# 10XGenomics/vartrix

Hardware: NVIDIA H100
Metric: reads_sw_scored_per_sec (higher is better)
Workload: dtype int16x2

## Files before the change

vartrix_b200/csrc/vtx_api.cu:

```cuda
#include "../../include/vartrix_b200.h"
#include "vtx_pipeline.cuh"
#include "vtx_sw.cuh"
#include "vtx_sw_band.cuh"
#include "vtx_inflate.cuh"
#include "vtx_stage.cuh"
#include "vtx_locus_stats.cuh"
#include "vtx_donors.cuh"

#include <nvtx3/nvToolsExt.h>

#include <algorithm>
#include <array>
#include <cstdarg>
#include <cstddef>
#include <cstdio>
#include <cstring>
#include <string>
#include <thread>
#include <vector>

using namespace vtx;

namespace {

thread_local std::string g_create_error;

struct Nvtx {
    explicit Nvtx(const char* name) { nvtxRangePushA(name); }
    ~Nvtx() { nvtxRangePop(); }
};
constexpr int kBandK = 6, kBandW = 20;

struct DBuf {
    void* p = nullptr;
    size_t cap = 0;
    DBuf() = default;
    DBuf(const DBuf&) = delete;
    DBuf& operator=(const DBuf&) = delete;
    ~DBuf() { release(); }
    cudaError_t release()
    {
        const cudaError_t e = p ? cudaFree(p) : cudaSuccess;
        p = nullptr; cap = 0;
        return e;
    }
    void swap(DBuf& o) { std::swap(p, o.p); std::swap(cap, o.cap); }
};

struct HostBuf {
    void* p = nullptr;
    HostBuf() = default;
    HostBuf(const HostBuf&) = delete;
    HostBuf& operator=(const HostBuf&) = delete;
    ~HostBuf() { release(); }
    void release() { if (p) cudaFreeHost(p); p = nullptr; }
    cudaError_t alloc(size_t bytes, unsigned flags = cudaHostAllocDefault)
    {
        release();
        const cudaError_t e = cudaHostAlloc(&p, bytes, flags);
        if (e != cudaSuccess) p = nullptr;
        return e;
    }
    template <typename T> T* as() const { return static_cast<T*>(p); }
};

constexpr int kResArrays = 7;
constexpr size_t kResEsz[kResArrays] = { 4, 4, 4, 4, 4, 8, 8 };

struct HostResults {
    HostBuf a[kResArrays];
    size_t cap = 0;
};

enum { EV_START = 0, EV_H2D, EV_C0, EV_PREP, EV_SW, EV_POST, EV_COUNT };

constexpr size_t kMaxCum = 4096;

struct TimeRec {
    cudaEvent_t ev[EV_COUNT] = {};
    bool had_h2d = false;
    uint64_t sw_launches = 0, launches = 0;
};

struct InSlot {
    DBuf locus_row, hap, ref_off, ref_len, alt_off, alt_len, cand_start, read_nib, read_off, read_len, cb_bytes,
        read_cb_off, read_cb_len, read_umi, cand_read;
    DBuf read_off4, read_len16, read_cb_key, cb_off_ex;
    cudaEvent_t copy_done = nullptr, free_ev = nullptr;
    bool used = false;
};

struct StageSlot {
    DBuf comp, desc, status, stream, entry, seg_count, seg_first, rec_off, rec_tid, rec_pos, rec_end, rec_fm, l_start, l_end,
        locus_row, hap, ref_off, ref_len, alt_off, alt_len, cand_count, cand_first, cand_rec, used, read_off, read_len,
        read_cb_off, read_cb_len, read_umi, cand_start, scalars, name_tab, lfilt;
    cudaEvent_t staged = nullptr, free_ev = nullptr;
    bool used_once = false;
};

}

struct vtx_ctx {
    vtx_config cfg{};
    int device = 0;
    int n_sm = 0;
    cudaStream_t stream = nullptr;
    bool own_stream = false;
    std::string err;

    DBuf bc_slot, bc_bytes, bc_off;
    DBuf bck_key, bck_idx;
    uint32_t bck_cap = 0;
    DBuf x_read_off, x_read_len, x_units, x_off4;
    DBuf band_scratch;
    DBuf inf_comp, inf_out, inf_desc, inf_status;
    bool inflate_attr_set = false;
    StageSlot sslot[2];
    uint64_t n_bam_submits = 0;
    cudaStream_t stage_stream = nullptr;
    DBuf bam_metrics;
    uint32_t min_base_quality = 0;
    DBuf stage_sums;
    bool locus_stats = false, submitted = false;
    DBuf lstats;
    size_t lstats_cap = 0;
    uint64_t stats_n = 0, stats_last_n = 0;
    HostBuf h_lstats;
    size_t h_lstats_cap = 0;
    bool donors = false;
    uint32_t n_donors = 0, donor_cols = 0, donor_last_cols = 0;
    uint64_t donor_rows = 0;
    donors::Tables donor_tab{};
    DBuf donor_dosage, donor_usable, donor_acc, donor_count, donor_start, donor_list;
    HostBuf h_donor;
    size_t h_donor_cap = 0;
    bool donor_valid = false;
    HostBuf h_stage;
    uint32_t bc_cap = 0, n_barcodes = 0;
    bool have_barcodes = false;

    InSlot slot[2];
    uint64_t n_submits = 0;
    cudaStream_t copy_stream = nullptr;
    DBuf read_col, keep, pidx, scan_sums, pair_read, pair_col, pair_umi, pair_locus, pair_start, tcount, tstart,
        pair_first, pair_cslot, pair_uslot, cslot_col, cslot_locus, uslot_cslot, ccnt, ucnt, keep2, oidx, tile_counters,
        scratch, pair_scores, d_metrics, d_res_n, big_list, slot_scratch;
    DBuf res[kResArrays];
    size_t res_cap = 0;
    size_t res_ub = 0;
    bool finished = true;
    HostResults h_res;
    HostBuf h_scalars;
    uint64_t last_n = 0;
    vtx_metrics last_metrics{};

    cudaStream_t fetch_stream = nullptr;
    HostBuf h_cum;
    unsigned long long* d_cum = nullptr;
    std::vector<TimeRec> trecs;
    size_t trec_used = 0;
    bool timing_valid = false;
    uint32_t last_tiles_nl = 0;
    bool last_tiles_valid = false;
    uint64_t t_pairs = 0;

    void* comm = nullptr;
    int rank = 0, n_ranks = 1;
    HostResults g_host;
    DBuf g_dev[kResArrays];
    DBuf g_counts;
    cudaStream_t comm_stream = nullptr;
    cudaEvent_t ev_counts = nullptr, ev_gather = nullptr, ev_results = nullptr;
    HostBuf h_counts;
    bool gather_pending = false;
    bool gather_guard = false;
    vtx_result g_out{};
};

namespace {

int set_err(vtx_ctx* c, int code, const char* fmt, ...)
{
    char buf[512];
    va_list ap; va_start(ap, fmt); vsnprintf(buf, sizeof(buf), fmt, ap); va_end(ap);
    if (c) c->err = buf; else g_create_error = buf;
    return code;
}

#define CK(call)                                                                                     \
    do {                                                                                             \
        cudaError_t e_ = (call);                                                                     \
        if (e_ != cudaSuccess)                                                                       \
            return set_err(ctx, VTX_E_CUDA, "%s failed: %s (%s:%d)", #call, cudaGetErrorString(e_), __FILE__, __LINE__); \
    } while (0)

int ensure(vtx_ctx* ctx, DBuf& b, size_t bytes)
{
    if (bytes <= b.cap) return VTX_OK;
    if (b.p) {
        CK(cudaStreamSynchronize(ctx->stream));
        if (ctx->copy_stream) CK(cudaStreamSynchronize(ctx->copy_stream));
        CK(b.release());
    }
    size_t want = bytes + bytes / 8 + 256;
    cudaError_t e = cudaMalloc(&b.p, want);
    if (e != cudaSuccess) { b.p = nullptr; return set_err(ctx, VTX_E_NOMEM, "cudaMalloc(%zu) failed: %s", want, cudaGetErrorString(e)); }
    b.cap = want;
    return VTX_OK;
}

#define ENS(buf, bytes) do { int rc_ = ensure(ctx, buf, (bytes)); if (rc_) return rc_; } while (0)

template <typename T> T* P(DBuf& b) { return static_cast<T*>(b.p); }

TimeRec* new_trec(vtx_ctx* ctx)
{
    if (ctx->finished) ctx->trec_used = 0;
    if (ctx->trec_used == ctx->trecs.size()) {
        TimeRec r;
        for (auto& e : r.ev) if (cudaEventCreate(&e) != cudaSuccess) return nullptr;
        ctx->trecs.push_back(r);
    }
    TimeRec* r = &ctx->trecs[ctx->trec_used++];
    r->had_h2d = false; r->sw_launches = 0; r->launches = 0;
    return r;
}

inline unsigned blocks_for(uint64_t n, unsigned threads) { return unsigned((n + threads - 1) / threads); }

int scan_u32(vtx_ctx* ctx, cudaStream_t st, DBuf& sums, const uint32_t* in, uint64_t n, uint32_t* out, uint64_t* launches)
{
    const unsigned nb = std::max(1u, blocks_for(n, kScanTile));
    ENS(sums, size_t(nb) * 4);
    vtx_k_scan_tiles<<<nb, kScanThreads, 0, st>>>(in, n, out, P<uint32_t>(sums));
    vtx_k_scan_sums<<<1, kScanThreads, 0, st>>>(P<uint32_t>(sums), nb, out + n);
    vtx_k_scan_add<<<nb, kScanThreads, 0, st>>>(out, n, P<uint32_t>(sums));
    if (launches) *launches += 3;
    CK(cudaGetLastError());
    return VTX_OK;
}

int launch_inflate(vtx_ctx* ctx, cudaStream_t st, const void* desc, uint32_t n, const void* comp, void* out, void* status,
                   uint32_t* cursor, int check_crc)
{
    using namespace inflate;
    if (!ctx->inflate_attr_set) {
        CK(cudaFuncSetAttribute(vtx_k_bgzf_inflate, cudaFuncAttributeMaxDynamicSharedMemorySize, int(inflate_smem_bytes())));
        ctx->inflate_attr_set = true;
    }
    const unsigned ctas = unsigned(std::min<uint64_t>((n + kInflateWarps - 1) / kInflateWarps, uint64_t(ctx->n_sm) * 6));
    vtx_k_bgzf_inflate<<<ctas, kInflateWarps * 32, inflate_smem_bytes(), st>>>(static_cast<const BlockDesc*>(desc), n,
        static_cast<const uint8_t*>(comp), static_cast<uint8_t*>(out), static_cast<int32_t*>(status), cursor, check_crc);
    CK(cudaGetLastError());
    return VTX_OK;
}

uint32_t want_mask(const vtx_ctx* ctx)
{
    const bool values_only = (ctx->cfg.flags & VTX_F_VALUES_ONLY) != 0;
    return values_only ? (ctx->cfg.mode == VTX_MODE_COVERAGE ? 0x63u : 0x23u) : 0x7Fu;
}

template <typename Buf> std::array<const void*, kResArrays> ptrs(const Buf (&b)[kResArrays])
{
    std::array<const void*, kResArrays> a;
    for (int i = 0; i < kResArrays; ++i) a[i] = b[i].p;
    return a;
}

void point_result(vtx_result* out, const std::array<const void*, kResArrays>& a, uint32_t want, uint64_t n, const vtx_metrics& m)
{
    auto u32 = [&](int i) { return (want >> i & 1) ? static_cast<const uint32_t*>(a[i]) : nullptr; };
    auto f64 = [&](int i) { return (want >> i & 1) ? static_cast<const double*>(a[i]) : nullptr; };
    out->n = n;
    out->row = u32(0); out->col = u32(1); out->ref_cnt = u32(2); out->alt_cnt = u32(3); out->unk_cnt = u32(4);
    out->val = f64(5); out->val2 = f64(6);
    out->metrics = m;
}

int ensure_host(vtx_ctx* ctx, HostResults& h, size_t n)
{
    if (n <= h.cap) return VTX_OK;
    const size_t ncap = n + n / 4 + 1024;
    const uint32_t want = want_mask(ctx);
    for (int i = 0; i < kResArrays; ++i) {
        h.a[i].release();
        if (!(want >> i & 1)) continue;
        const cudaError_t e = h.a[i].alloc(ncap * kResEsz[i]);
        if (e != cudaSuccess) { h.cap = 0; return set_err(ctx, VTX_E_NOMEM, "pinned result alloc failed: %s", cudaGetErrorString(e)); }
    }
    h.cap = ncap;
    return VTX_OK;
}

int copy_results(vtx_ctx* ctx, HostResults& h, const std::array<const void*, kResArrays>& src, size_t from, size_t to, cudaStream_t st)
{
    const uint32_t want = want_mask(ctx);
    for (int i = 0; i < kResArrays; ++i)
        if ((want >> i & 1) && src[i])
            CK(cudaMemcpyAsync(h.a[i].as<uint8_t>() + from * kResEsz[i], static_cast<const uint8_t*>(src[i]) + from * kResEsz[i],
                               (to - from) * kResEsz[i], cudaMemcpyDeviceToHost, st));
    return VTX_OK;
}

struct DevBatch {
    uint32_t n_loci = 0; uint32_t n_reads = 0; uint64_t n_cand = 0;
    const uint32_t* locus_row; const uint8_t* hap; const uint32_t *ref_off, *ref_len, *alt_off, *alt_len;
    const uint64_t* cand_start; const uint8_t* read_nib; const uint64_t* read_off; const uint32_t* read_len;
    const uint8_t* cb_bytes; const uint32_t* read_cb_off; const uint16_t* read_cb_len; const uint64_t* read_umi;
    const uint32_t* cand_read;
    const uint64_t* read_cb_key = nullptr; const uint32_t* cb_off_ex = nullptr;
    bool have_shapes = false;
    uint64_t shapes = 0;
    uint32_t max_read_len = 0, max_hap_len = 0;
    uint64_t max_depth = ~0ull;
    const uint32_t* lfilt = nullptr;
};

int launch_sw(vtx_ctx* ctx, void (*kern)(SwArgs), int threads, size_t smem, const SwArgs& a, uint64_t* launches,
              const char* name, int cls)
{
    CK(cudaFuncSetAttribute(kern, cudaFuncAttributeMaxDynamicSharedMemorySize, int(smem)));
    int per_sm = 0;
    CK(cudaOccupancyMaxActiveBlocksPerMultiprocessor(&per_sm, kern, threads, smem));
    if (per_sm < 1) {
        if (cls < 0) return set_err(ctx, VTX_E_CUDA, "%s does not fit on an SM (smem %zu)", name, smem);
        return set_err(ctx, VTX_E_CUDA, "%s %d does not fit on an SM (smem %zu)", name, cls, smem);
    }
    kern<<<ctx->n_sm * per_sm, threads, smem, ctx->stream>>>(a);
    CK(cudaGetLastError());
    ++*launches;
    return VTX_OK;
}

template <int CLS> int launch_sw_class(vtx_ctx* ctx, const SwArgs& a, uint64_t* launches)
{
    return launch_sw(ctx, vtx_k_sw_pairs<CLS>, TileClass<CLS>::THREADS,
                     sw_warp_bytes<CLS>(a.mcap, a.multi) * (TileClass<CLS>::THREADS / 32), a, launches,
                     "SW kernel class", CLS);
}
template <int SCLS> int launch_sw_split(vtx_ctx* ctx, const SwArgs& a, uint64_t* launches)
{
    return launch_sw(ctx, vtx_k_sw_split<SCLS>, SplitClass<SCLS>::THREADS,
                     split_warp_bytes<SCLS>(a.mcap) * (SplitClass<SCLS>::THREADS / 32), a, launches,
                     "split SW kernel", SCLS);
}
template <int W, int S, bool SHARED> int launch_sw_fold(vtx_ctx* ctx, const SwArgs& a, uint64_t* launches)
{
    return launch_sw(ctx, vtx_k_sw_fold<W, S, SHARED>, W * 32, fold_cta_bytes<W, S>(), a, launches, "folded SW kernel", -1);
}

int run_sw(vtx_ctx* ctx, const DevBatch& b, uint32_t n_pairs_ub, const uint32_t* pair_slot, uint32_t* counters,
           uint32_t* pair_scores, uint64_t* launches, uint64_t* sw_launches, TimeRec* tr)
{
    const uint32_t nl = b.n_loci;
    ENS(ctx->tcount, size_t(kNumClasses) * (nl + 1) * 4);
    ENS(ctx->tstart, size_t(kNumClasses) * (nl + 1) * 4);
    ENS(ctx->tile_counters, 64);
    const SwAllow allow = allowed_kernels(ctx->cfg.flags, b.max_read_len, b.max_hap_len);
    vtx_k_locus_prep<<<blocks_for(uint64_t(nl) * 32, 256), 256, 0, ctx->stream>>>(
        nl, b.hap, b.ref_off, b.ref_len, b.alt_off, b.alt_len, P<uint32_t>(ctx->pair_start), P<uint32_t>(ctx->pair_read), b.read_len,
        allow, b.max_read_len, b.max_hap_len, P<unsigned long long>(ctx->d_metrics) + 4, P<uint32_t>(ctx->tcount));
    ++*launches;
    vtx_k_scan_rows<<<kNumClasses, kScanThreads, 0, ctx->stream>>>(P<uint32_t>(ctx->tcount), P<uint32_t>(ctx->tstart), nl, nl + 1);
    ++*launches;
    CK(cudaGetLastError());
    CK(cudaMemsetAsync(ctx->tile_counters.p, 0, 64, ctx->stream));
    ctx->last_tiles_nl = nl;
    ctx->last_tiles_valid = true;
    if (tr) CK(cudaEventRecord(tr->ev[EV_PREP], ctx->stream));

    SwArgs a{};
    a.hap_bytes = b.hap; a.ref_off = b.ref_off; a.ref_len = b.ref_len; a.alt_off = b.alt_off; a.alt_len = b.alt_len;
    a.read_nib = b.read_nib; a.read_off = b.read_off; a.read_len = b.read_len;
    a.pair_read = P<uint32_t>(ctx->pair_read); a.pair_start = P<uint32_t>(ctx->pair_start);
    a.n_loci = nl; a.pair_slot = pair_slot; a.counters = counters; a.pair_scores = pair_scores;
    a.min_score = ctx->cfg.min_score;
    int mcap = int(std::min<uint32_t>(b.max_read_len, kFastMaxRead));
    mcap = std::max(2, (mcap + 1) & ~1);
    a.mcap = mcap;
    a.k64k = 65536u;
    a.multi = allow.multi;
    a.max_hap = b.max_hap_len;

    uint64_t before = *launches;
    if (ctx->cfg.band_mode == VTX_BAND_MODEL) {
        BandArgs ba{};
        ba.sw = a; ba.n_pairs_ub = n_pairs_ub; ba.k = ctx->cfg.band_k; ba.w = ctx->cfg.band_w;
        ba.max_read = std::max<uint32_t>(b.max_read_len, 8); ba.max_hap = std::max<uint32_t>(b.max_hap_len, 8);
        const uint64_t all_hits = uint64_t(ba.max_read) * ba.max_hap;
        ba.hit_cap = uint32_t(std::min<uint64_t>(all_hits, uint64_t(1) << 20));
        ba.hit_cap = std::min<uint32_t>(ba.hit_cap, 65535u * 16u);
        const size_t wb = band_warp_bytes(ba.max_read, ba.max_hap, ba.hit_cap);
        size_t warps = size_t(ctx->n_sm) * 16;
        const size_t budget = size_t(4) << 30;
        if (warps * wb > budget) warps = std::max<size_t>(size_t(ctx->n_sm), budget / wb);
        warps = std::max<size_t>(warps & ~size_t(3), 4);
        ENS(ctx->band_scratch, warps * wb);
        ba.scratch = P<uint8_t>(ctx->band_scratch);
        if (ba.max_hap >= 65536u || ba.max_read >= 65536u) return set_err(ctx, VTX_E_UNSUPPORTED, "band model: reads and windows must be shorter than 65536");
        ba.overflow = P<unsigned long long>(ctx->d_metrics) + 5;
        ba.bounds_violated = P<unsigned long long>(ctx->d_metrics) + 4;
        ba.cursor = P<uint32_t>(ctx->tile_counters);
        vtx_k_sw_band<<<unsigned(warps / (kBandThreads / 32)), kBandThreads, 0, ctx->stream>>>(ba);
        CK(cudaGetLastError());
        ++*launches;
        *sw_launches += *launches - before;
        return VTX_OK;
    }
    const uint32_t mask = b.have_shapes ? host_class_mask(b.shapes, allow, b.max_read_len) : device_class_mask(allow, b.max_hap_len);
    for (int c = 0; c < kNumClasses; ++c) {
        if (!(mask >> c & 1u)) continue;
        a.tile_start = P<uint32_t>(ctx->tstart) + size_t(c) * (nl + 1);
        a.tile_counter = P<uint32_t>(ctx->tile_counters) + c;
        int rc = VTX_OK;
        switch (c) {
        case 0: rc = launch_sw_class<0>(ctx, a, launches); break;
        case 1: rc = launch_sw_class<1>(ctx, a, launches); break;
        case 2: rc = launch_sw_class<2>(ctx, a, launches); break;
        case 3: rc = launch_sw_class<3>(ctx, a, launches); break;
        case kSlowClass: {
            const unsigned blocks = unsigned(ctx->n_sm) * 4, threads = 128;
            const size_t warps = size_t(blocks) * threads / 32;
            ENS(ctx->scratch, warps * (size_t(b.max_hap_len) + 1) * 32 * 4);
            a.scratch = P<uint32_t>(ctx->scratch);
            vtx_k_sw_generic<<<blocks, threads, 0, ctx->stream>>>(a);
            CK(cudaGetLastError());
            ++*launches;
            break;
        }
        case kSplitClass0: rc = launch_sw_split<0>(ctx, a, launches); break;
        case kSplitClass0 + 1: rc = launch_sw_split<1>(ctx, a, launches); break;
        case kFoldClass: {
            const bool deep = uint64_t(n_pairs_ub) >= uint64_t(kFoldDeepDepth) * nl;
            rc = deep ? launch_sw_fold<kFoldDeepWarps, kFoldDeepSlots, true>(ctx, a, launches)
                      : launch_sw_fold<kFoldShallowWarps, kFoldShallowWarps, false>(ctx, a, launches);
            break;
        }
        }
        if (rc) return rc;
    }
    *sw_launches += *launches - before;
    return VTX_OK;
}

int grow_results(vtx_ctx* ctx, size_t need)
{
    if (need <= ctx->res_cap) return VTX_OK;
    const size_t ncap = need + need / 4 + 1024;
    for (int i = 0; i < kResArrays; ++i) {
        DBuf& b = ctx->res[i];
        DBuf nb;
        cudaError_t e = cudaMalloc(&nb.p, ncap * kResEsz[i]);
        if (e != cudaSuccess) { nb.p = nullptr; return set_err(ctx, VTX_E_NOMEM, "result cudaMalloc(%zu) failed: %s", ncap * kResEsz[i], cudaGetErrorString(e)); }
        nb.cap = ncap * kResEsz[i];
        if (b.p && ctx->res_ub && !ctx->finished)
            CK(cudaMemcpyAsync(nb.p, b.p, ctx->res_ub * kResEsz[i], cudaMemcpyDeviceToDevice, ctx->stream));
        if (b.p) {
            CK(cudaStreamSynchronize(ctx->stream));
            if (ctx->fetch_stream) CK(cudaStreamSynchronize(ctx->fetch_stream));
            if (ctx->comm_stream) CK(cudaStreamSynchronize(ctx->comm_stream));
            CK(b.release());
        }
        b.swap(nb);
    }
    ctx->res_cap = ncap;
    return VTX_OK;
}

static_assert(sizeof(vtx_locus_stats) == sizeof(uint32_t) * lstats::kFields, "vtx_locus_stats is the kernel's record");

int grow_stats(vtx_ctx* ctx, size_t need)
{
    if (need <= ctx->lstats_cap) return VTX_OK;
    const size_t ncap = need + need / 2 + 1024;
    DBuf nb;
    const cudaError_t e = cudaMalloc(&nb.p, ncap * sizeof(vtx_locus_stats));
    if (e != cudaSuccess) { nb.p = nullptr; return set_err(ctx, VTX_E_NOMEM, "locus statistics cudaMalloc failed: %s", cudaGetErrorString(e)); }
    nb.cap = ncap * sizeof(vtx_locus_stats);
    if (ctx->lstats.p) {
        if (ctx->stats_n) CK(cudaMemcpyAsync(nb.p, ctx->lstats.p, ctx->stats_n * sizeof(vtx_locus_stats), cudaMemcpyDeviceToDevice, ctx->stream));
        CK(cudaStreamSynchronize(ctx->stream));
        CK(ctx->lstats.release());
    }
    ctx->lstats.swap(nb);
    ctx->lstats_cap = ncap;
    return VTX_OK;
}

int launch_locus_stats(vtx_ctx* ctx, const DevBatch& b, bool have_pairs, uint64_t* launches)
{
    const int use_umi = ctx->cfg.use_umi ? 1 : 0;
    lstats::Inputs in{ b.cand_start, b.cand_read, P<int32_t>(ctx->read_col), use_umi ? b.read_umi : nullptr,
                       have_pairs ? P<uint32_t>(ctx->pair_start) : nullptr, use_umi ? P<uint32_t>(ctx->ucnt) : nullptr,
                       P<uint32_t>(ctx->ccnt), P<uint32_t>(ctx->cslot_col), b.locus_row, b.lfilt };
    const unsigned grid = std::min<unsigned>(b.n_loci, unsigned(ctx->n_sm) * 16);
    lstats::vtx_k_locus_stats<<<grid, lstats::kStatsThreads, 0, ctx->stream>>>(in, b.n_loci, P<uint32_t>(ctx->lstats) + ctx->stats_n * lstats::kFields);
    CK(cudaGetLastError());
    ctx->stats_n += b.n_loci;
    ++*launches;
    return VTX_OK;
}

size_t donor_acc_bytes(uint32_t cols, uint32_t n_hyp) { return size_t(cols) * (size_t(n_hyp) + 3) * 8 + 8; }

int launch_donors(vtx_ctx* ctx, const DevBatch& b, uint32_t n_slots_ub, const uint32_t* n_slots, uint64_t* launches)
{
    using namespace donors;
    cudaStream_t st = ctx->stream;
    const uint32_t H = n_hyp(ctx->n_donors), nc = ctx->donor_cols;
    Inputs in{ P<uint32_t>(ctx->cslot_col), P<uint32_t>(ctx->cslot_locus), b.locus_row, P<uint32_t>(ctx->ccnt),
               P<uint8_t>(ctx->donor_dosage), P<uint8_t>(ctx->donor_usable), ctx->donor_rows, nc, ctx->n_donors, H, ctx->donor_tab };
    int64_t* ll = P<int64_t>(ctx->donor_acc);
    uint64_t* cnt = reinterpret_cast<uint64_t*>(ll + size_t(nc) * H);
    unsigned long long* bad = reinterpret_cast<unsigned long long*>(cnt + size_t(nc) * 3);
    const unsigned grid = std::max(1u, std::min(blocks_for(std::max<uint64_t>(n_slots_ub, b.n_loci), kDonorThreads), unsigned(ctx->n_sm) * 16));
    ENS(ctx->donor_count, (size_t(nc) + 1) * 4);
    CK(cudaMemsetAsync(ctx->donor_count.p, 0, size_t(nc) * 4, st));
    vtx_k_donor_count<<<grid, kDonorThreads, 0, st>>>(in, n_slots_ub, n_slots, b.n_loci, P<uint32_t>(ctx->donor_count), bad);
    CK(cudaGetLastError());
    ++*launches;
    if (!n_slots) return VTX_OK;
    ENS(ctx->donor_start, (size_t(nc) + 1) * 4);
    ENS(ctx->donor_list, size_t(n_slots_ub) * 4 + 4);
    int rc = scan_u32(ctx, st, ctx->scan_sums, P<uint32_t>(ctx->donor_count), nc, P<uint32_t>(ctx->donor_start), launches);
    if (rc) return rc;
    CK(cudaMemsetAsync(ctx->donor_count.p, 0, size_t(nc) * 4, st));
    vtx_k_donor_scatter<<<grid, kDonorThreads, 0, st>>>(in, n_slots_ub, n_slots, P<uint32_t>(ctx->donor_start),
                                                        P<uint32_t>(ctx->donor_count), P<uint32_t>(ctx->donor_list));
    const unsigned ll_grid = std::max(1u, std::min(blocks_for(uint64_t(nc) * 32, kDonorThreads), unsigned(ctx->n_sm) * 8));
    const uint32_t* cs = P<uint32_t>(ctx->donor_start);
    const uint32_t* lst = P<uint32_t>(ctx->donor_list);
    if (H <= 32) vtx_k_donor_ll<1><<<ll_grid, kDonorThreads, 0, st>>>(in, cs, lst, ll, cnt);
    else if (H <= 64) vtx_k_donor_ll<2><<<ll_grid, kDonorThreads, 0, st>>>(in, cs, lst, ll, cnt);
    else if (H <= 160) vtx_k_donor_ll<5><<<ll_grid, kDonorThreads, 0, st>>>(in, cs, lst, ll, cnt);
    else if (H <= 288) vtx_k_donor_ll<9><<<ll_grid, kDonorThreads, 0, st>>>(in, cs, lst, ll, cnt);
    else vtx_k_donor_ll<17><<<ll_grid, kDonorThreads, 0, st>>>(in, cs, lst, ll, cnt);
    CK(cudaGetLastError());
    *launches += 2;
    return VTX_OK;
}

int process_batch(vtx_ctx* ctx, const DevBatch& b, TimeRec* tr)
{
    const uint64_t nc = b.n_cand;
    const uint32_t nl = b.n_loci, nr = b.n_reads;
    const int use_umi = ctx->cfg.use_umi ? 1 : 0;
    uint64_t launches = 0, sw_launches = 0;
    cudaStream_t st = ctx->stream;

    if (ctx->finished) {
        CK(cudaMemsetAsync(ctx->d_res_n.p, 0, 8, st));
        CK(cudaMemsetAsync(ctx->d_metrics.p, 0, 48, st));
        ctx->res_ub = 0;
        ctx->stats_n = 0;
        if (ctx->donors) {
            ctx->donor_cols = ctx->n_barcodes;
            const size_t bytes = donor_acc_bytes(ctx->donor_cols, donors::n_hyp(ctx->n_donors));
            ENS(ctx->donor_acc, bytes);
            CK(cudaMemsetAsync(ctx->donor_acc.p, 0, bytes, st));
        }
        ctx->finished = false;
    }
    int rc = grow_results(ctx, ctx->res_ub + nc);
    if (rc) return rc;
    const bool stats = ctx->locus_stats && nl > 0;
    if (stats && (rc = grow_stats(ctx, ctx->stats_n + nl))) return rc;
    const bool donor = ctx->donors && nl > 0;

    const size_t ncp = size_t(nc) + 1;
    ENS(ctx->read_col, size_t(nr ? nr : 1) * 4);
    ENS(ctx->keep, ncp * 4); ENS(ctx->pidx, ncp * 4);
    ENS(ctx->pair_read, ncp * 4); ENS(ctx->pair_col, ncp * 4);
    if (use_umi) ENS(ctx->pair_umi, ncp * 8);
    ENS(ctx->pair_start, size_t(nl + 1) * 4);
    ENS(ctx->pair_first, ncp);
    ENS(ctx->pair_cslot, ncp * 4); ENS(ctx->cslot_col, ncp * 4); ENS(ctx->cslot_locus, ncp * 4);
    ENS(ctx->ccnt, ncp * 16);
    if (use_umi) { ENS(ctx->pair_uslot, ncp * 4); ENS(ctx->uslot_cslot, ncp * 4); ENS(ctx->ucnt, ncp * 16); }
    ENS(ctx->keep2, ncp * 4); ENS(ctx->oidx, ncp * 4);
    uint32_t* pair_scores = nullptr;
    if (ctx->cfg.flags & VTX_F_KEEP_SCORES) { ENS(ctx->pair_scores, ncp * 4); pair_scores = P<uint32_t>(ctx->pair_scores); }

    if (nl == 0 || nc == 0) {
        if (ctx->d_cum && ctx->trec_used - 1 < kMaxCum)
            vtx_k_bump<<<1, 32, 0, st>>>(P<unsigned long long>(ctx->d_res_n), nullptr, ctx->d_cum + (ctx->trec_used - 1));
        CK(cudaEventRecord(tr->ev[EV_PREP], st)); CK(cudaEventRecord(tr->ev[EV_SW], st));
        if (stats) {
            if ((rc = launch_locus_stats(ctx, b, false, &launches))) return rc;
            tr->launches = launches;
        }
        if (donor) {
            if ((rc = launch_donors(ctx, b, 0, nullptr, &launches))) return rc;
            tr->launches = launches;
        }
        CK(cudaEventRecord(tr->ev[EV_POST], st));
        ctx->timing_valid = true;
        return VTX_OK;
    }

    Nvtx r_prep("vtx: prep kernels (CB lookup, filter, compaction, slots)");
    BarcodeTable tab{ P<int32_t>(ctx->bc_slot), ctx->bc_cap - 1, P<uint8_t>(ctx->bc_bytes), P<uint32_t>(ctx->bc_off) };
    if (b.read_cb_key) {
        BarcodeKeyTable kt{ P<uint64_t>(ctx->bck_key), P<uint32_t>(ctx->bck_idx), ctx->bck_cap - 1 };
        vtx_k_cb_lookup_key<<<blocks_for(nr, 256), 256, 0, st>>>(tab, kt, nr, b.read_cb_key, b.cb_bytes, b.cb_off_ex, P<int32_t>(ctx->read_col));
    } else {
        vtx_k_cb_lookup<<<blocks_for(nr, 256), 256, 0, st>>>(tab, nr, b.cb_bytes, b.read_cb_off, b.read_cb_len, P<int32_t>(ctx->read_col));
    }
    vtx_k_cand_filter<<<blocks_for(nc, 256), 256, 0, st>>>(nc, b.cand_read, P<int32_t>(ctx->read_col), b.read_umi, use_umi,
                                                           P<uint32_t>(ctx->keep), P<unsigned long long>(ctx->d_metrics));
    launches += 2;
    rc = scan_u32(ctx, st, ctx->scan_sums, P<uint32_t>(ctx->keep), nc, P<uint32_t>(ctx->pidx), &launches);
    if (rc) return rc;
    vtx_k_compact<<<blocks_for(nc, 256), 256, 0, st>>>(nc, b.cand_read, P<uint32_t>(ctx->keep), P<uint32_t>(ctx->pidx),
                                                       P<int32_t>(ctx->read_col), b.read_umi, use_umi, P<uint32_t>(ctx->pair_read),
                                                       P<uint32_t>(ctx->pair_col), P<uint64_t>(ctx->pair_umi));
    vtx_k_pair_start<<<blocks_for(nl + 1, 256), 256, 0, st>>>(nl, b.cand_start, P<uint32_t>(ctx->pidx), P<uint32_t>(ctx->pair_start));
    launches += 2;
    const uint32_t* n_pairs_ptr = P<uint32_t>(ctx->pidx) + nc;

    ENS(ctx->big_list, size_t(nc / kSlotSmallMax + 2) * 4);
    CK(cudaMemsetAsync(ctx->big_list.p, 0, 4, st));
    if (b.max_depth > kSlotSmallMax) ENS(ctx->slot_scratch, size_t(kSlotBigWords) * nc * 4);
    CK(cudaMemsetAsync(ctx->cslot_col.p, 0xFF, size_t(nc) * 4, st));
    CK(cudaMemsetAsync(ctx->ccnt.p, 0, size_t(nc) * 16, st));
    if (use_umi) {
        CK(cudaMemsetAsync(ctx->uslot_cslot.p, 0xFF, size_t(nc) * 4, st));
        CK(cudaMemsetAsync(ctx->ucnt.p, 0, size_t(nc) * 16, st));
    }
    vtx_k_slots<<<std::min<uint32_t>(nl, 65535u * 8), kSlotThreads, 0, st>>>(
        nl, P<uint32_t>(ctx->pair_start), P<uint32_t>(ctx->pair_col), P<uint64_t>(ctx->pair_umi), use_umi,
        P<uint8_t>(ctx->pair_first), P<uint32_t>(ctx->pair_cslot), P<uint32_t>(ctx->pair_uslot),
        P<uint32_t>(ctx->cslot_col), P<uint32_t>(ctx->cslot_locus), P<uint32_t>(ctx->uslot_cslot), P<uint32_t>(ctx->big_list));
    ++launches;
    if (nc > kSlotSmallMax) {
        vtx_k_slots_big<<<ctx->n_sm, kSlotBigThreads, 0, st>>>(
            P<uint32_t>(ctx->big_list), P<uint32_t>(ctx->pair_start), P<uint32_t>(ctx->pair_col), P<uint64_t>(ctx->pair_umi), use_umi,
            P<uint32_t>(ctx->slot_scratch), P<uint32_t>(ctx->pair_cslot), P<uint32_t>(ctx->pair_uslot), P<uint32_t>(ctx->cslot_col),
            P<uint32_t>(ctx->cslot_locus), P<uint32_t>(ctx->uslot_cslot));
        ++launches;
    }
    CK(cudaGetLastError());

    nvtxRangePop(); nvtxRangePushA("vtx: Smith-Waterman kernels");
    rc = run_sw(ctx, b, uint32_t(nc), use_umi ? P<uint32_t>(ctx->pair_uslot) : P<uint32_t>(ctx->pair_cslot),
                use_umi ? P<uint32_t>(ctx->ucnt) : P<uint32_t>(ctx->ccnt), pair_scores, &launches, &sw_launches, tr);
    if (rc) return rc;
    CK(cudaEventRecord(tr->ev[EV_SW], st));

    nvtxRangePop(); nvtxRangePushA("vtx: post kernels (UMI collapse, finalize, emit)");
    if (use_umi) {
        vtx_k_umi_collapse<<<blocks_for(nc, 256), 256, 0, st>>>(uint32_t(nc), n_pairs_ptr, P<uint32_t>(ctx->uslot_cslot),
                                                                P<uint32_t>(ctx->ucnt), P<uint32_t>(ctx->ccnt));
        ++launches;
    }
    if (stats && (rc = launch_locus_stats(ctx, b, true, &launches))) return rc;
    if (donor && (rc = launch_donors(ctx, b, uint32_t(nc), n_pairs_ptr, &launches))) return rc;
    vtx_k_finalize<<<blocks_for(nc, 256), 256, 0, st>>>(uint32_t(nc), n_pairs_ptr, ctx->cfg.mode, P<uint32_t>(ctx->cslot_col),
                                                        P<uint32_t>(ctx->ccnt), P<uint32_t>(ctx->keep2));
    ++launches;
    rc = scan_u32(ctx, st, ctx->scan_sums, P<uint32_t>(ctx->keep2), nc, P<uint32_t>(ctx->oidx), &launches);
    if (rc) return rc;
    if (ctx->gather_guard) {
        CK(cudaStreamWaitEvent(st, ctx->ev_gather, 0));
        ctx->gather_guard = false;
    }
    ResultArrays out{ P<uint32_t>(ctx->res[0]), P<uint32_t>(ctx->res[1]), P<uint32_t>(ctx->res[2]), P<uint32_t>(ctx->res[3]),
                      P<uint32_t>(ctx->res[4]), P<double>(ctx->res[5]), P<double>(ctx->res[6]) };
    vtx_k_emit<<<blocks_for(nc, 256), 256, 0, st>>>(uint32_t(nc), ctx->cfg.mode, P<uint32_t>(ctx->keep2), P<uint32_t>(ctx->oidx),
                                                    P<unsigned long long>(ctx->d_res_n), P<uint32_t>(ctx->cslot_col),
                                                    P<uint32_t>(ctx->cslot_locus), b.locus_row, P<uint32_t>(ctx->ccnt), out);
    const size_t sub_idx = ctx->trec_used - 1;
    vtx_k_bump<<<1, 32, 0, st>>>(P<unsigned long long>(ctx->d_res_n), P<uint32_t>(ctx->oidx) + nc,
                                 (ctx->d_cum && sub_idx < kMaxCum) ? ctx->d_cum + sub_idx : nullptr);
    launches += 2;
    CK(cudaGetLastError());
    CK(cudaEventRecord(tr->ev[EV_POST], st));
    ctx->res_ub += nc;
    ctx->timing_valid = true;
    tr->sw_launches = sw_launches;
    tr->launches = launches;
    return VTX_OK;
}

struct BatchView {
    uint32_t n_loci = 0, n_reads = 0; uint64_t n_cand = 0;
    const uint32_t *locus_row = nullptr, *ref_off = nullptr, *ref_len = nullptr, *alt_off = nullptr, *alt_len = nullptr;
    const uint64_t* cand_start = nullptr; const uint8_t* hap = nullptr; uint64_t hap_len = 0;
    const uint8_t* read_nib = nullptr; uint64_t nib_len = 0; const uint8_t* cb_bytes = nullptr; uint64_t cb_bytes_len = 0;
    const uint64_t* read_off = nullptr; const uint32_t* read_len = nullptr; const uint32_t* cb_off = nullptr; const uint16_t* cb_len = nullptr;
    const uint32_t* read_off4 = nullptr; const uint16_t* read_len16 = nullptr; const uint64_t* cb_key = nullptr;
    uint32_t n_exotic = 0; const uint32_t* cb_off_ex = nullptr;
    const uint64_t* umi = nullptr; const uint32_t* cand_read = nullptr;
    bool v2 = false;
};

BatchView view_of(const vtx_batch* b)
{
    BatchView v;
    v.n_loci = b->n_loci; v.n_reads = b->n_reads; v.n_cand = b->n_cand;
    v.locus_row = b->locus_row; v.ref_off = b->ref_off; v.ref_len = b->ref_len; v.alt_off = b->alt_off; v.alt_len = b->alt_len;
    v.cand_start = b->cand_start; v.hap = b->hap_bytes; v.hap_len = b->hap_bytes_len;
    v.read_nib = b->read_nib; v.nib_len = b->read_nib_len; v.cb_bytes = b->cb_bytes; v.cb_bytes_len = b->cb_bytes_len;
    v.read_off = b->read_off; v.read_len = b->read_len; v.cb_off = b->read_cb_off; v.cb_len = b->read_cb_len;
    v.umi = b->read_umi_key; v.cand_read = b->cand_read;
    return v;
}
BatchView view_of(const vtx_batch2* b)
{
    BatchView v;
    v.v2 = true;
    v.n_loci = b->n_loci; v.n_reads = b->n_reads; v.n_cand = b->n_cand;
    v.locus_row = b->locus_row; v.ref_off = b->ref_off; v.ref_len = b->ref_len; v.alt_off = b->alt_off; v.alt_len = b->alt_len;
    v.cand_start = b->cand_start; v.hap = b->hap_bytes; v.hap_len = b->hap_bytes_len;
    v.read_nib = b->read_nib; v.nib_len = b->read_nib_len; v.cb_bytes = b->cb_bytes;
    v.read_off4 = b->read_off4; v.read_len16 = b->read_len; v.cb_key = b->read_cb_key; v.n_exotic = b->n_exotic_cb; v.cb_off_ex = b->cb_off;
    v.umi = b->read_umi_key; v.cand_read = b->cand_read;
    return v;
}

DevBatch dev_batch_of(const BatchView& v, uint32_t max_read_len, uint32_t max_hap_len)
{
    DevBatch d{};
    d.n_loci = v.n_loci; d.n_reads = v.n_reads; d.n_cand = v.n_cand;
    d.locus_row = v.locus_row; d.hap = v.hap; d.ref_off = v.ref_off; d.ref_len = v.ref_len; d.alt_off = v.alt_off; d.alt_len = v.alt_len;
    d.cand_start = v.cand_start; d.read_nib = v.read_nib; d.cb_bytes = v.cb_bytes;
    d.read_off = v.read_off; d.read_len = v.read_len; d.read_cb_off = v.cb_off; d.read_cb_len = v.cb_len;
    d.read_cb_key = v.cb_key; d.cb_off_ex = v.cb_off_ex;
    d.read_umi = v.umi; d.cand_read = v.cand_read;
    d.max_read_len = max_read_len; d.max_hap_len = max_hap_len;
    return d;
}

int validate_batch(vtx_ctx* ctx, const BatchView& b)
{
    if (b.n_cand >= 0xFFFFFFF0ull) return set_err(ctx, VTX_E_INVALID, "n_cand %llu exceeds 2^32 per shard; split the shard", (unsigned long long)b.n_cand);
    if (b.n_loci && (!b.locus_row || !b.ref_off || !b.ref_len || !b.alt_off || !b.alt_len || !b.cand_start))
        return set_err(ctx, VTX_E_INVALID, "locus arrays missing");
    if (b.n_reads) {
        const bool reads_ok = b.v2 ? (b.read_len16 && b.cb_key) : (b.read_off && b.read_len && b.cb_off && b.cb_len);
        if (!reads_ok || (!b.umi && ctx->cfg.use_umi)) return set_err(ctx, VTX_E_INVALID, "read arrays missing");
    }
    if (b.v2 && b.n_exotic && !b.cb_off_ex) return set_err(ctx, VTX_E_INVALID, "cb_off missing for the exotic cell tags");
    if (b.n_cand && !b.cand_read && !(b.v2 && b.n_cand == b.n_reads)) return set_err(ctx, VTX_E_INVALID, "cand_read missing (NULL means identity and needs n_cand == n_reads in a vtx_batch2)");
    if (b.hap_len >= 0xFFFFFFFFull) return set_err(ctx, VTX_E_INVALID, "haplotype pool exceeds 4 GiB; split the shard");
    if (b.v2 && b.nib_len >= (uint64_t(1) << 34)) return set_err(ctx, VTX_E_INVALID, "read pool exceeds 16 GiB; split the shard");
    return VTX_OK;
}

int scan_host_batch(vtx_ctx* ctx, const BatchView& b, uint32_t* max_read, uint32_t* max_hap, bool check_cands,
                    uint64_t* max_depth = nullptr, uint64_t* shapes_seen = nullptr)
{
    if (check_cands && b.n_loci && (b.cand_start[0] != 0 || b.cand_start[b.n_loci] != b.n_cand))
        return set_err(ctx, VTX_E_INVALID, "cand_start must span [0, n_cand]");
    if (check_cands && !b.n_loci && b.n_cand) return set_err(ctx, VTX_E_INVALID, "candidates without loci");
    if (b.v2 && b.n_exotic) {
        for (uint32_t i = 0; i < b.n_exotic; ++i)
            if (b.cb_off_ex[i] > b.cb_off_ex[i + 1]) return set_err(ctx, VTX_E_INVALID, "cb_off must be ascending (exotic tag %u)", i);
    }
    const bool scan_cands = check_cands && b.cand_read != nullptr;
    const uint64_t work = uint64_t(b.n_reads) + (scan_cands ? b.n_cand : 0) + uint64_t(b.n_loci) * 64;
    unsigned nt = std::min<unsigned>(8u, std::max(1u, std::thread::hardware_concurrency()));
    if (work < (1u << 16)) nt = 1;
    struct Part { uint32_t mr = 0, mh = 0; uint64_t md = 0, units = 0; int bad = 0; uint64_t where = 0, seen = 0; };
    std::vector<Part> parts(nt);
    auto worker = [&](unsigned t) {
        Part& pt = parts[t];
        auto flag = [&](int code, uint64_t where) { if (!pt.bad) { pt.bad = code; pt.where = where; } };
        const uint32_t l0 = uint32_t(uint64_t(b.n_loci) * t / nt), l1 = uint32_t(uint64_t(b.n_loci) * (t + 1) / nt);
        for (uint32_t l = l0; l < l1; ++l) {
            if ((b.ref_off[l] & 15) || (b.alt_off[l] & 15)) { flag(10, l); continue; }
            if (uint64_t(b.ref_off[l]) + b.ref_len[l] > b.hap_len || uint64_t(b.alt_off[l]) + b.alt_len[l] > b.hap_len) { flag(11, l); continue; }
            if (l && b.locus_row[l] <= b.locus_row[l - 1]) flag(12, l);
            if (check_cands && b.cand_start[l] > b.cand_start[l + 1]) flag(13, l);
            if (check_cands) pt.md = std::max<uint64_t>(pt.md, b.cand_start[l + 1] - b.cand_start[l]);
            pt.mh = std::max(pt.mh, std::max(b.ref_len[l], b.alt_len[l]));
            if (shapes_seen) pt.seen |= uint64_t(1) << shape_key(window_shape(b.hap + b.ref_off[l], b.ref_len[l], b.hap + b.alt_off[l], b.alt_len[l]));
        }
        const uint32_t r0 = uint32_t(uint64_t(b.n_reads) * t / nt), r1 = uint32_t(uint64_t(b.n_reads) * (t + 1) / nt);
        for (uint32_t r = r0; r < r1; ++r) {
            uint32_t len;
            if (b.v2) {
                len = b.read_len16[r];
                const uint64_t nb = (uint64_t(len) + 1) / 2;
                if (b.read_off4) { if (uint64_t(b.read_off4[r]) * 4 + nb > b.nib_len) flag(2, r); }
                else pt.units += (nb + 3) / 4;
                const uint64_t k = b.cb_key[r];
                if (k != VTX_NO_CB_KEY && (k & VTX_CB_EXOTIC) && (k & ~VTX_CB_EXOTIC) >= b.n_exotic) flag(3, r);
                else if (k != VTX_NO_CB_KEY && !(k & VTX_CB_EXOTIC) && (k >> 60)) flag(6, r);
            } else {
                len = b.read_len[r];
                if (b.read_off[r] & 15) flag(1, r);
                else if (b.read_off[r] + (uint64_t(len) + 1) / 2 > b.nib_len) flag(2, r);
                else if (b.cb_off[r] != VTX_NO_CB && uint64_t(b.cb_off[r]) + b.cb_len[r] > b.cb_bytes_len) flag(3, r);
            }
            if (b.umi && b.umi[r] != VTX_NO_UMI && b.umi[r] > VTX_UMI_KEY_MAX) flag(4, r);
            pt.mr = std::max(pt.mr, len);
        }
        if (scan_cands) {
            const uint64_t c0 = b.n_cand * t / nt, c1 = b.n_cand * (t + 1) / nt;
            uint32_t worst = 0;
            for (uint64_t c = c0; c < c1; ++c) worst = std::max(worst, b.cand_read[c]);
            if (c1 > c0 && worst >= b.n_reads) flag(5, c0);
        }
    };
    if (nt == 1) worker(0);
    else {
        std::vector<std::thread> th;
        for (unsigned t = 1; t < nt; ++t) th.emplace_back(worker, t);
        worker(0);
        for (auto& x : th) x.join();
    }
    uint32_t mr = 0, mh = 0;
    uint64_t md = 0, units = 0;
    for (const Part& pt : parts) {
        mr = std::max(mr, pt.mr); mh = std::max(mh, pt.mh); md = std::max(md, pt.md); units += pt.units;
        if (shapes_seen) *shapes_seen |= pt.seen;
        const unsigned long long w = (unsigned long long)pt.where;
        switch (pt.bad) {
        case 1: return set_err(ctx, VTX_E_INVALID, "read %llu: read_off must be a multiple of 16", w);
        case 2: return set_err(ctx, VTX_E_INVALID, "read %llu outside read_nib", w);
        case 3: return set_err(ctx, VTX_E_INVALID, "read %llu: CB outside cb_bytes", w);
        case 4: return set_err(ctx, VTX_E_INVALID, "read %llu: UMI key exceeds VTX_UMI_KEY_MAX", w);
        case 5: return set_err(ctx, VTX_E_INVALID, "cand_read out of range near candidate %llu", w);
        case 6: return set_err(ctx, VTX_E_INVALID, "read %llu: read_cb_key is not a vtx_pack_cb code", w);
        case 10: return set_err(ctx, VTX_E_INVALID, "locus %llu: haplotype offsets must be multiples of 16", w);
        case 11: return set_err(ctx, VTX_E_INVALID, "locus %llu: haplotype window outside hap_bytes", w);
        case 12: return set_err(ctx, VTX_E_INVALID, "locus_row must be strictly ascending (locus %llu)", w);
        case 13: return set_err(ctx, VTX_E_INVALID, "cand_start must be ascending (locus %llu)", w);
        default: break;
        }
    }
    if (b.v2 && !b.read_off4 && units * 4 > b.nib_len) return set_err(ctx, VTX_E_INVALID, "dense read pool is shorter than the reads it should hold");
    if (mr > uint32_t(kMaxRead)) return set_err(ctx, VTX_E_UNSUPPORTED, "reads longer than %d bases (biased int16 DP) are not supported (%u)", kMaxRead, mr);
    *max_read = mr; *max_hap = mh;
    if (max_depth) *max_depth = md;
    return VTX_OK;
}

int upload(vtx_ctx* ctx, DBuf& d, const void* h, size_t bytes)
{
    ENS(d, bytes ? bytes : 16);
    if (bytes) CK(cudaMemcpyAsync(d.p, h, bytes, cudaMemcpyHostToDevice, ctx->copy_stream));
    return VTX_OK;
}

#define UP(buf, ptr, bytes) do { int rc_ = upload(ctx, buf, ptr, (bytes)); if (rc_) return rc_; } while (0)

int claim_slot(vtx_ctx* ctx, InSlot** out)
{
    InSlot* sl = &ctx->slot[ctx->n_submits & 1];
    ++ctx->n_submits;
    if (sl->used) CK(cudaStreamWaitEvent(ctx->copy_stream, sl->free_ev, 0));
    sl->used = true;
    *out = sl;
    return VTX_OK;
}

int upload_loci(vtx_ctx* ctx, InSlot* sl, const BatchView& h, DevBatch& d)
{
    const size_t nl = h.n_loci;
    UP(sl->locus_row, h.locus_row, nl * 4);
    UP(sl->hap, h.hap, h.hap_len);
    UP(sl->ref_off, h.ref_off, nl * 4); UP(sl->ref_len, h.ref_len, nl * 4);
    UP(sl->alt_off, h.alt_off, nl * 4); UP(sl->alt_len, h.alt_len, nl * 4);
    d.n_loci = h.n_loci; d.n_reads = h.n_reads; d.n_cand = h.n_cand;
    d.locus_row = P<uint32_t>(sl->locus_row); d.hap = P<uint8_t>(sl->hap);
    d.ref_off = P<uint32_t>(sl->ref_off); d.ref_len = P<uint32_t>(sl->ref_len);
    d.alt_off = P<uint32_t>(sl->alt_off); d.alt_len = P<uint32_t>(sl->alt_len);
    return VTX_OK;
}

int upload_common(vtx_ctx* ctx, InSlot* sl, const BatchView& h, DevBatch& d)
{
    int rc = upload_loci(ctx, sl, h, d);
    if (rc) return rc;
    UP(sl->read_nib, h.read_nib, h.nib_len);
    UP(sl->read_off, h.read_off, size_t(h.n_reads) * 8); UP(sl->read_len, h.read_len, size_t(h.n_reads) * 4);
    d.read_nib = P<uint8_t>(sl->read_nib); d.read_off = P<uint64_t>(sl->read_off); d.read_len = P<uint32_t>(sl->read_len);
    return VTX_OK;
}

int upload_batch(vtx_ctx* ctx, InSlot* sl, const BatchView& h, DevBatch& d)
{
    int rc = upload_common(ctx, sl, h, d);
    if (rc) return rc;
    const size_t nr = h.n_reads;
    UP(sl->cand_start, h.cand_start, size_t(h.n_loci + 1) * 8);
    UP(sl->cb_bytes, h.cb_bytes, h.cb_bytes_len);
    UP(sl->read_cb_off, h.cb_off, nr * 4); UP(sl->read_cb_len, h.cb_len, nr * 2);
    if (h.umi) UP(sl->read_umi, h.umi, nr * 8);
    UP(sl->cand_read, h.cand_read, size_t(h.n_cand) * 4);
    d.cand_start = P<uint64_t>(sl->cand_start); d.cb_bytes = P<uint8_t>(sl->cb_bytes);
    d.read_cb_off = P<uint32_t>(sl->read_cb_off); d.read_cb_len = P<uint16_t>(sl->read_cb_len);
    d.read_umi = h.umi ? P<uint64_t>(sl->read_umi) : nullptr; d.cand_read = P<uint32_t>(sl->cand_read);
    return VTX_OK;
}

int upload_batch2(vtx_ctx* ctx, InSlot* sl, const BatchView& h, DevBatch& d)
{
    int rc = upload_loci(ctx, sl, h, d);
    if (rc) return rc;
    const size_t nr = h.n_reads;
    UP(sl->cand_start, h.cand_start, size_t(h.n_loci + 1) * 8);
    UP(sl->read_nib, h.read_nib, h.nib_len);
    if (h.read_off4) UP(sl->read_off4, h.read_off4, nr * 4);
    UP(sl->read_len16, h.read_len16, nr * 2);
    UP(sl->read_cb_key, h.cb_key, nr * 8);
    if (h.n_exotic) { UP(sl->cb_bytes, h.cb_bytes, h.cb_off_ex[h.n_exotic]); UP(sl->cb_off_ex, h.cb_off_ex, size_t(h.n_exotic + 1) * 4); }
    if (h.umi) UP(sl->read_umi, h.umi, nr * 8);
    if (h.cand_read) UP(sl->cand_read, h.cand_read, size_t(h.n_cand) * 4);
    d.cand_start = P<uint64_t>(sl->cand_start); d.read_nib = P<uint8_t>(sl->read_nib);
    d.read_cb_key = P<uint64_t>(sl->read_cb_key);
    d.cb_bytes = h.n_exotic ? P<uint8_t>(sl->cb_bytes) : nullptr; d.cb_off_ex = h.n_exotic ? P<uint32_t>(sl->cb_off_ex) : nullptr;
    d.read_umi = h.umi ? P<uint64_t>(sl->read_umi) : nullptr;
    d.cand_read = h.cand_read ? P<uint32_t>(sl->cand_read) : nullptr;
    return VTX_OK;
}

int expand_reads(vtx_ctx* ctx, uint32_t nr, const uint16_t* d_len16, const uint32_t* d_off4, DevBatch& d)
{
    ENS(ctx->x_read_off, size_t(nr ? nr : 1) * 8); ENS(ctx->x_read_len, size_t(nr ? nr : 1) * 4);
    if (nr) {
        if (!d_off4) {
            ENS(ctx->x_units, size_t(nr) * 4); ENS(ctx->x_off4, size_t(nr + 1) * 4);
            vtx_k_read_units<<<blocks_for(nr, 256), 256, 0, ctx->stream>>>(nr, d_len16, P<uint32_t>(ctx->x_units));
            int rc = scan_u32(ctx, ctx->stream, ctx->scan_sums, P<uint32_t>(ctx->x_units), nr, P<uint32_t>(ctx->x_off4), nullptr);
            if (rc) return rc;
            d_off4 = P<uint32_t>(ctx->x_off4);
        }
        vtx_k_expand_reads<<<blocks_for(nr, 256), 256, 0, ctx->stream>>>(nr, d_len16, d_off4, P<uint64_t>(ctx->x_read_off), P<uint32_t>(ctx->x_read_len));
        CK(cudaGetLastError());
    }
    d.read_off = P<uint64_t>(ctx->x_read_off); d.read_len = P<uint32_t>(ctx->x_read_len);
    return VTX_OK;
}

template <typename Check>
int begin_submit(vtx_ctx* ctx, const void* batch, const char* fn, const char* what, Check check, uint32_t max_read_len, TimeRec** tr)
{
    if (!ctx->have_barcodes) return set_err(ctx, VTX_E_STATE, "vtx_set_barcodes must be called before %s", fn);
    if (!batch) return set_err(ctx, VTX_E_INVALID, "%s is NULL", what);
    int rc = check();
    if (rc) return rc;
    if (max_read_len > uint32_t(kMaxRead)) return set_err(ctx, VTX_E_UNSUPPORTED, "reads longer than %d bases are not supported", kMaxRead);
    CK(cudaSetDevice(ctx->device));
    *tr = new_trec(ctx);
    if (!*tr) return set_err(ctx, VTX_E_CUDA, "cudaEventCreate failed");
    ctx->submitted = true;
    return VTX_OK;
}

template <typename Batch>
int submit_host(vtx_ctx* ctx, const Batch* hb, const char* fn)
{
    Nvtx nvtx_range(fn);
    BatchView h;
    TimeRec* tr = nullptr;
    int rc = begin_submit(ctx, hb, fn, "batch", [&] { h = view_of(hb); return validate_batch(ctx, h); }, 0, &tr);
    if (rc) return rc;
    InSlot* sl = nullptr;
    rc = claim_slot(ctx, &sl);
    if (rc) return rc;
    DevBatch d{};
    CK(cudaEventRecord(tr->ev[EV_START], ctx->copy_stream));
    rc = h.v2 ? upload_batch2(ctx, sl, h, d) : upload_batch(ctx, sl, h, d);
    if (rc) return rc;
    CK(cudaEventRecord(tr->ev[EV_H2D], ctx->copy_stream));
    CK(cudaEventRecord(sl->copy_done, ctx->copy_stream));
    tr->had_h2d = true;
    { Nvtx r_val("vtx: validate host batch (copies in flight)");
      rc = scan_host_batch(ctx, h, &d.max_read_len, &d.max_hap_len, true, &d.max_depth, &d.shapes); }
    if (rc) { cudaStreamSynchronize(ctx->copy_stream); --ctx->trec_used; return rc; }
    d.have_shapes = true;
    CK(cudaStreamWaitEvent(ctx->stream, sl->copy_done, 0));
    CK(cudaEventRecord(tr->ev[EV_C0], ctx->stream));
    if (h.v2) {
        rc = expand_reads(ctx, h.n_reads, P<uint16_t>(sl->read_len16), h.read_off4 ? P<uint32_t>(sl->read_off4) : nullptr, d);
        if (rc) return rc;
    }
    rc = process_batch(ctx, d, tr);
    if (rc) return rc;
    CK(cudaEventRecord(sl->free_ev, ctx->stream));
    return VTX_OK;
}

template <typename Batch>
int submit_resident(vtx_ctx* ctx, const Batch* db, const char* fn, uint32_t max_read_len, uint32_t max_hap_len)
{
    BatchView v;
    TimeRec* tr = nullptr;
    int rc = begin_submit(ctx, db, fn, "batch", [&] { v = view_of(db); return validate_batch(ctx, v); }, max_read_len, &tr);
    if (rc) return rc;
    DevBatch d = dev_batch_of(v, max_read_len, max_hap_len);
    CK(cudaEventRecord(tr->ev[EV_C0], ctx->stream));
    if (v.v2) {
        rc = expand_reads(ctx, v.n_reads, v.read_len16, v.read_off4, d);
        if (rc) return rc;
    }
    return process_batch(ctx, d, tr);
}

void comm_destroy(vtx_ctx* ctx);

}

extern "C" {

int vtx_abi_version(void) { return VTX_ABI_VERSION; }

const char* vtx_last_error(const vtx_ctx* ctx) { return ctx ? ctx->err.c_str() : g_create_error.c_str(); }

int vtx_create(const vtx_config* cfg, vtx_ctx** out)
{
    vtx_ctx* ctx = nullptr;
    if (!cfg || !out) return set_err(nullptr, VTX_E_INVALID, "vtx_create: NULL argument");
    *out = nullptr;
    if (cfg->match != kMatch || cfg->mismatch != kMismatch || cfg->gap_open != kGapOpen || cfg->gap_extend != kGapExtend)
        return set_err(nullptr, VTX_E_UNSUPPORTED, "scoring constants are compiled in: match %d mismatch %d gap_open %d gap_extend %d (main.rs:35-38)",
                       kMatch, kMismatch, kGapOpen, kGapExtend);
    if (cfg->mode < 0 || cfg->mode > 2) return set_err(nullptr, VTX_E_INVALID, "unknown mode %d", cfg->mode);
    if ((cfg->flags & VTX_F_NAME_KEYS) && !cfg->use_umi)
        return set_err(nullptr, VTX_E_INVALID, "VTX_F_NAME_KEYS collapses reads through the UMI path: it needs use_umi");
    if (cfg->band_mode != VTX_BAND_FULL && cfg->band_mode != VTX_BAND_MODEL) return set_err(nullptr, VTX_E_INVALID, "unknown band_mode %d", cfg->band_mode);
    if (cfg->band_k < 0 || cfg->band_k > 8 || cfg->band_w < 0 || cfg->band_w > 4096)
        return set_err(nullptr, VTX_E_UNSUPPORTED, "band constants out of range: K %d (1..8; 0 = %d), W %d (0 = %d; main.rs:33-34)", cfg->band_k, kBandK, cfg->band_w, kBandW);
    int n_dev = 0;
    cudaError_t e = cudaGetDeviceCount(&n_dev);
    if (e != cudaSuccess || n_dev == 0)
        return set_err(nullptr, VTX_E_CUDA, "no CUDA device available (%s); vartrix_b200 has no CPU fallback", cudaGetErrorString(e));
    if (cfg->device < 0 || cfg->device >= n_dev) return set_err(nullptr, VTX_E_INVALID, "device %d out of range (%d devices)", cfg->device, n_dev);
    CK(cudaSetDevice(cfg->device));
    ctx = new vtx_ctx();
    ctx->cfg = *cfg; ctx->device = cfg->device;
    if (ctx->cfg.band_k == 0) ctx->cfg.band_k = kBandK;
    if (ctx->cfg.band_w == 0) ctx->cfg.band_w = kBandW;
    cudaDeviceProp prop{};
    cudaError_t pe = cudaGetDeviceProperties(&prop, cfg->device);
    if (pe != cudaSuccess) { g_create_error = cudaGetErrorString(pe); delete ctx; return VTX_E_CUDA; }
    if (prop.major != 9 || prop.minor != 0) {
        delete ctx;
        return set_err(nullptr, VTX_E_UNSUPPORTED, "vartrix_b200 is built for sm_90a (H100, compute capability 9.0); device %d is %d.%d",
                       cfg->device, prop.major, prop.minor);
    }
    ctx->n_sm = prop.multiProcessorCount;
    if (cfg->stream) { ctx->stream = static_cast<cudaStream_t>(cfg->stream); ctx->own_stream = false; }
    else {
        pe = cudaStreamCreateWithFlags(&ctx->stream, cudaStreamNonBlocking);
        if (pe != cudaSuccess) { g_create_error = cudaGetErrorString(pe); delete ctx; return VTX_E_CUDA; }
        ctx->own_stream = true;
    }
    pe = cudaStreamCreateWithFlags(&ctx->copy_stream, cudaStreamNonBlocking);
    if (pe != cudaSuccess) { g_create_error = cudaGetErrorString(pe); vtx_destroy(ctx); return VTX_E_CUDA; }
    cudaStreamCreateWithFlags(&ctx->fetch_stream, cudaStreamNonBlocking);
    if (ctx->h_cum.alloc(kMaxCum * 8, cudaHostAllocMapped) == cudaSuccess) {
        if (cudaHostGetDevicePointer(reinterpret_cast<void**>(&ctx->d_cum), ctx->h_cum.p, 0) != cudaSuccess) ctx->d_cum = nullptr;
    } else cudaGetLastError();
    for (auto& sl : ctx->slot) {
        cudaEventCreateWithFlags(&sl.copy_done, cudaEventDisableTiming);
        cudaEventCreateWithFlags(&sl.free_ev, cudaEventDisableTiming);
    }
    bool ok = cudaMalloc(&ctx->d_metrics.p, 64) == cudaSuccess && cudaMalloc(&ctx->d_res_n.p, 64) == cudaSuccess &&
              ctx->h_scalars.alloc(64) == cudaSuccess;
    if (!ok) { g_create_error = "allocation of context scalars failed"; vtx_destroy(ctx); return VTX_E_NOMEM; }
    ctx->d_metrics.cap = 64; ctx->d_res_n.cap = 64;
    cudaMemsetAsync(ctx->d_metrics.p, 0, 64, ctx->stream);
    cudaMemsetAsync(ctx->d_res_n.p, 0, 64, ctx->stream);
    *out = ctx;
    return VTX_OK;
}

void vtx_destroy(vtx_ctx* ctx)
{
    if (!ctx) return;
    cudaSetDevice(ctx->device);
    for (cudaStream_t s : { ctx->stream, ctx->comm_stream, ctx->copy_stream, ctx->stage_stream, ctx->fetch_stream })
        if (s) cudaStreamSynchronize(s);
    comm_destroy(ctx);
    for (auto& sl : ctx->slot)
        for (cudaEvent_t e : { sl.copy_done, sl.free_ev }) if (e) cudaEventDestroy(e);
    for (auto& ss : ctx->sslot)
        for (cudaEvent_t e : { ss.staged, ss.free_ev }) if (e) cudaEventDestroy(e);
    for (auto& tr : ctx->trecs) for (auto& ev : tr.ev) if (ev) cudaEventDestroy(ev);
    for (cudaEvent_t e : { ctx->ev_counts, ctx->ev_gather, ctx->ev_results }) if (e) cudaEventDestroy(e);
    for (cudaStream_t s : { ctx->stage_stream, ctx->comm_stream, ctx->copy_stream, ctx->fetch_stream }) if (s) cudaStreamDestroy(s);
    if (ctx->own_stream && ctx->stream) cudaStreamDestroy(ctx->stream);
    delete ctx;
}

int vtx_host_alloc(void** out, uint64_t bytes)
{
    if (!out) return VTX_E_INVALID;
    cudaError_t e = cudaHostAlloc(out, bytes ? bytes : 16, cudaHostAllocDefault);
    if (e != cudaSuccess) { g_create_error = cudaGetErrorString(e); *out = nullptr; return VTX_E_NOMEM; }
    return VTX_OK;
}

int vtx_host_free(void* p) { return cudaFreeHost(p) == cudaSuccess ? VTX_OK : VTX_E_CUDA; }

int vtx_set_barcodes(vtx_ctx* ctx, const uint8_t* bytes, const uint32_t* off, uint32_t n)
{
    if (!ctx) return VTX_E_INVALID;
    if (!off || (n && !bytes && off[n] > 0)) return set_err(ctx, VTX_E_INVALID, "vtx_set_barcodes: NULL argument");
    if (n == 0) return set_err(ctx, VTX_E_INVALID, "Loaded 0 barcodes (main.rs:712-715)");
    CK(cudaSetDevice(ctx->device));
    uint32_t cap = 16;
    while (cap < 2ull * n + 1) cap <<= 1;
    std::vector<int32_t> slot(cap, -1);
    for (uint32_t i = 0; i < n; ++i) {
        if (off[i + 1] < off[i]) return set_err(ctx, VTX_E_INVALID, "barcode offsets must be ascending");
        const uint32_t len = off[i + 1] - off[i];
        if (len > 0xFFFF) return set_err(ctx, VTX_E_INVALID, "barcode %u longer than 65535 bytes", i);
        uint32_t h = uint32_t(fnv1a64(bytes + off[i], len)) & (cap - 1);
        for (;;) {
            const int32_t s = slot[h];
            if (s < 0) { slot[h] = int32_t(i); break; }
            const uint32_t l2 = off[s + 1] - off[s];
            if (l2 == len && memcmp(bytes + off[s], bytes + off[i], len) == 0)
                return set_err(ctx, VTX_E_INVALID, "duplicate barcode at index %u (first seen at %d); dedup first (main.rs:706-709)", i, s);
            h = (h + 1) & (cap - 1);
        }
    }
    std::vector<uint64_t> kkey(cap, kNoCbKey);
    std::vector<uint32_t> kidx(cap, 0);
    for (uint32_t i = 0; i < n; ++i) {
        const uint64_t k = stage::pack_cb(bytes + off[i], off[i + 1] - off[i]);
        if (k == kNoCbKey) continue;
        uint32_t h = uint32_t(mix64(k)) & (cap - 1);
        while (kkey[h] != kNoCbKey) h = (h + 1) & (cap - 1);
        kkey[h] = k; kidx[h] = i;
    }
    UP(ctx->bc_slot, slot.data(), size_t(cap) * 4);
    UP(ctx->bc_bytes, bytes, off[n]);
    UP(ctx->bc_off, off, size_t(n + 1) * 4);
    UP(ctx->bck_key, kkey.data(), size_t(cap) * 8);
    UP(ctx->bck_idx, kidx.data(), size_t(cap) * 4);
    CK(cudaStreamSynchronize(ctx->copy_stream));
    ctx->bc_cap = cap; ctx->bck_cap = cap; ctx->n_barcodes = n; ctx->have_barcodes = true;
    return VTX_OK;
}

int vtx_submit(vtx_ctx* ctx, const vtx_batch* hb)
{
    if (!ctx) return VTX_E_INVALID;
    return submit_host(ctx, hb, "vtx_submit");
}

int vtx_submit_device_ex(vtx_ctx* ctx, const vtx_batch* db, uint32_t max_read_len, uint32_t max_hap_len)
{
    if (!ctx) return VTX_E_INVALID;
    return submit_resident(ctx, db, "vtx_submit_device", max_read_len, max_hap_len);
}

int vtx_submit_device(vtx_ctx* ctx, const vtx_batch* db)
{
    return vtx_submit_device_ex(ctx, db, kFastMaxRead, class_max_n(kNumFastClasses - 1));
}

int vtx_submit2(vtx_ctx* ctx, const vtx_batch2* hb)
{
    if (!ctx) return VTX_E_INVALID;
    return submit_host(ctx, hb, "vtx_submit2");
}

int vtx_submit2_device(vtx_ctx* ctx, const vtx_batch2* db, uint32_t max_read_len, uint32_t max_hap_len)
{
    if (!ctx) return VTX_E_INVALID;
    return submit_resident(ctx, db, "vtx_submit2_device", max_read_len, max_hap_len);
}
int vtx_bgzf_inflate(vtx_ctx* ctx, const vtx_bgzf_block* blocks, uint32_t n_blocks, const uint8_t* comp, uint64_t comp_len,
                     uint8_t* out, uint64_t out_len, int32_t* status, uint32_t flags)
{
    if (!ctx) return VTX_E_INVALID;
    Nvtx nvtx_range("vtx_bgzf_inflate");
    if (n_blocks == 0) return VTX_OK;
    if (!blocks || !comp || !status || (!out && out_len)) return set_err(ctx, VTX_E_INVALID, "vtx_bgzf_inflate: NULL argument");
    static_assert(sizeof(vtx_bgzf_block) == sizeof(inflate::BlockDesc), "descriptor layouts must agree");
    for (uint32_t i = 0; i < n_blocks; ++i) {
        const vtx_bgzf_block& b = blocks[i];
        if ((b.in_off & 3) || b.in_off + b.in_len + 8 > comp_len + 8 || b.in_off + b.in_len > comp_len)
            return set_err(ctx, VTX_E_INVALID, "vtx_bgzf_inflate: member %u: payload must start on a 4-byte boundary inside comp", i);
        if (b.out_len > 65536u || b.out_off + b.out_len > out_len) return set_err(ctx, VTX_E_INVALID, "vtx_bgzf_inflate: member %u: output outside out / ISIZE above 64 KiB", i);
    }
    CK(cudaSetDevice(ctx->device));
    cudaStream_t st = ctx->stream;
    ENS(ctx->inf_comp, size_t(comp_len) + 16); ENS(ctx->inf_out, size_t(out_len) + 16);
    ENS(ctx->inf_desc, size_t(n_blocks) * sizeof(vtx_bgzf_block)); ENS(ctx->inf_status, size_t(n_blocks) * 4 + 16);
    ENS(ctx->tile_counters, 64);
    CK(cudaMemsetAsync(static_cast<uint8_t*>(ctx->inf_comp.p) + comp_len, 0, 16, st));
    CK(cudaMemcpyAsync(ctx->inf_comp.p, comp, comp_len, cudaMemcpyHostToDevice, st));
    CK(cudaMemcpyAsync(ctx->inf_desc.p, blocks, size_t(n_blocks) * sizeof(vtx_bgzf_block), cudaMemcpyHostToDevice, st));
    CK(cudaMemsetAsync(ctx->tile_counters.p, 0, 64, st));
    if (int rc = launch_inflate(ctx, st, ctx->inf_desc.p, n_blocks, ctx->inf_comp.p, ctx->inf_out.p, ctx->inf_status.p,
                                P<uint32_t>(ctx->tile_counters), (flags & VTX_BGZF_CHECK_CRC) ? 1 : 0)) return rc;
    if (out_len) CK(cudaMemcpyAsync(out, ctx->inf_out.p, out_len, cudaMemcpyDeviceToHost, st));
    CK(cudaMemcpyAsync(status, ctx->inf_status.p, size_t(n_blocks) * 4, cudaMemcpyDeviceToHost, st));
    CK(cudaStreamSynchronize(st));
    for (uint32_t i = 0; i < n_blocks; ++i)
        if (status[i] != 0) return set_err(ctx, VTX_E_INVALID, "vtx_bgzf_inflate: member %u failed with decoder status %d (corrupt data)", i, status[i]);
    return VTX_OK;
}


int vtx_submit_bam(vtx_ctx* ctx, const vtx_bam_shard* sh)
{
    if (!ctx) return VTX_E_INVALID;
    Nvtx nvtx_range("vtx_submit_bam");
    uint32_t nl = 0, nm = 0, ne = 0, max_hap = 0;
    uint64_t stream_len = 0;
    auto check = [&]() -> int {
        nl = sh->n_loci; nm = sh->n_members; ne = sh->n_entry;
        if (nl && (!sh->locus_row || !sh->locus_start || !sh->locus_end || !sh->ref_off || !sh->ref_len || !sh->alt_off || !sh->alt_len))
            return set_err(ctx, VTX_E_INVALID, "vtx_submit_bam: locus arrays missing");
        if (nm && (!sh->members || !sh->comp)) return set_err(ctx, VTX_E_INVALID, "vtx_submit_bam: members missing");
        if ((ne == 1) || (ne && !sh->entry_off)) return set_err(ctx, VTX_E_INVALID, "vtx_submit_bam: entry_off needs at least a start and an end");
        if (sh->hap_bytes_len >= 0xFFFFFFFFull) return set_err(ctx, VTX_E_INVALID, "haplotype pool exceeds 4 GiB; split the shard");
        for (uint32_t i = 0; i < nm; ++i) {
            const vtx_bgzf_block& b = sh->members[i];
            if ((b.in_off & 3) || b.in_off + b.in_len > sh->comp_len || b.out_len > 65536u || b.out_off != stream_len)
                return set_err(ctx, VTX_E_INVALID, "vtx_submit_bam: member %u: payload on a 4-byte boundary inside comp, out_off = running sum of out_len", i);
            stream_len += b.out_len;
        }
        if (stream_len >= 0xFFFFFFFFull) return set_err(ctx, VTX_E_INVALID, "vtx_submit_bam: more than 4 GiB of records in one shard; split the shard");
        for (uint32_t i = 0; i < ne; ++i)
            if (sh->entry_off[i] > stream_len || (i && sh->entry_off[i] <= sh->entry_off[i - 1])) return set_err(ctx, VTX_E_INVALID, "vtx_submit_bam: entry_off must ascend inside the stream");
        for (uint32_t l = 0; l < nl; ++l) {
            if ((sh->ref_off[l] & 15) || (sh->alt_off[l] & 15) || uint64_t(sh->ref_off[l]) + sh->ref_len[l] > sh->hap_bytes_len ||
                uint64_t(sh->alt_off[l]) + sh->alt_len[l] > sh->hap_bytes_len) return set_err(ctx, VTX_E_INVALID, "vtx_submit_bam: locus %u: bad haplotype window", l);
            if (l && (sh->locus_row[l] <= sh->locus_row[l - 1])) return set_err(ctx, VTX_E_INVALID, "locus_row must be strictly ascending (locus %u)", l);
            max_hap = std::max(max_hap, std::max(sh->ref_len[l], sh->alt_len[l]));
        }
        return VTX_OK;
    };
    TimeRec* tr = nullptr;
    int rc = begin_submit(ctx, sh, "vtx_submit_bam", "shard", check, 0, &tr);
    if (rc) return rc;
    if (!ctx->stage_stream) {
        CK(cudaStreamCreateWithFlags(&ctx->stage_stream, cudaStreamNonBlocking));
        for (auto& ss : ctx->sslot) { CK(cudaEventCreateWithFlags(&ss.staged, cudaEventDisableTiming)); CK(cudaEventCreateWithFlags(&ss.free_ev, cudaEventDisableTiming)); }
        ENS(ctx->bam_metrics, sizeof(stage::LocusMetrics));
        CK(cudaMemsetAsync(ctx->bam_metrics.p, 0, sizeof(stage::LocusMetrics), ctx->stage_stream));
        CK(ctx->h_stage.alloc(256));
    }
    cudaStream_t ss = ctx->stage_stream;
    StageSlot& sl = ctx->sslot[ctx->n_bam_submits & 1];
    ++ctx->n_bam_submits;
    if (sl.used_once) CK(cudaEventSynchronize(sl.free_ev));
    sl.used_once = true;
    auto fail_out = [&](int code) { --ctx->trec_used; sl.used_once = false; return code; };

    auto up = [&](DBuf& d, const void* h, size_t bytes) -> int {
        int rc = ensure(ctx, d, bytes ? bytes + 16 : 16);
        if (rc) return rc;
        if (bytes && cudaMemcpyAsync(d.p, h, bytes, cudaMemcpyHostToDevice, ss) != cudaSuccess) return set_err(ctx, VTX_E_CUDA, "cudaMemcpyAsync failed in vtx_submit_bam");
        return VTX_OK;
    };
    CK(cudaEventRecord(tr->ev[EV_START], ss));
    if ((rc = up(sl.comp, sh->comp, sh->comp_len)) || (rc = up(sl.desc, sh->members, size_t(nm) * sizeof(vtx_bgzf_block))) ||
        (rc = up(sl.entry, sh->entry_off, size_t(ne) * 8)) || (rc = up(sl.l_start, sh->locus_start, size_t(nl) * 8)) ||
        (rc = up(sl.l_end, sh->locus_end, size_t(nl) * 8)) || (rc = up(sl.locus_row, sh->locus_row, size_t(nl) * 4)) ||
        (rc = up(sl.hap, sh->hap_bytes, sh->hap_bytes_len)) || (rc = up(sl.ref_off, sh->ref_off, size_t(nl) * 4)) ||
        (rc = up(sl.ref_len, sh->ref_len, size_t(nl) * 4)) || (rc = up(sl.alt_off, sh->alt_off, size_t(nl) * 4)) ||
        (rc = up(sl.alt_len, sh->alt_len, size_t(nl) * 4))) return fail_out(rc);
    CK(cudaMemsetAsync(static_cast<uint8_t*>(sl.comp.p) + sh->comp_len, 0, 16, ss));
    CK(cudaEventRecord(tr->ev[EV_H2D], ss));
    tr->had_h2d = true;
    ENS(sl.stream, size_t(stream_len) + stage::kWalkWindow + 64);
    ENS(sl.status, size_t(nm) * 4 + 16); ENS(sl.scalars, 256);
    uint32_t* d_sc = P<uint32_t>(sl.scalars);
    CK(cudaMemsetAsync(sl.scalars.p, 0, 256, ss));
    if (nm && (rc = launch_inflate(ctx, ss, sl.desc.p, nm, sl.comp.p, sl.stream.p, sl.status.p, d_sc, 1))) return fail_out(rc);
    stage::Params sp{};
    sp.s = P<uint8_t>(sl.stream); sp.s_len = stream_len; sp.tid = sh->tid;
    sp.mapq_min = sh->mapq; sp.primary_only = sh->primary_only != 0; sp.no_duplicates = sh->no_duplicates != 0;
    sp.min_base_quality = ctx->min_base_quality;
    const bool name_keys = (ctx->cfg.flags & VTX_F_NAME_KEYS) != 0;
    sp.want_umi = ctx->cfg.use_umi && !name_keys ? 1 : 0; sp.tag0 = uint8_t(sh->bam_tag[0]); sp.tag1 = uint8_t(sh->bam_tag[1]);
    const uint32_t n_seg = ne ? ne - 1 : 0;
    ENS(sl.seg_count, size_t(n_seg + 1) * 4); ENS(sl.seg_first, size_t(n_seg + 2) * 4);
    uint32_t n_rec = 0;
    std::vector<int32_t> h_status(nm);
    if (n_seg) {
        stage::vtx_k_walk<<<blocks_for(n_seg, stage::kWalkWarps), stage::kWalkWarps * 32, 0, ss>>>(sp, n_seg, P<uint64_t>(sl.entry), 0, P<uint32_t>(sl.seg_count), nullptr, nullptr, d_sc + 1);
        rc = scan_u32(ctx, ss, ctx->stage_sums, P<uint32_t>(sl.seg_count), n_seg, P<uint32_t>(sl.seg_first), nullptr);
        if (rc) return fail_out(rc);
    }
    uint32_t* hs = ctx->h_stage.as<uint32_t>();
    if (n_seg) CK(cudaMemcpyAsync(hs, P<uint32_t>(sl.seg_first) + n_seg, 4, cudaMemcpyDeviceToHost, ss)); else hs[0] = 0;
    CK(cudaMemcpyAsync(hs + 1, d_sc + 1, 4, cudaMemcpyDeviceToHost, ss));
    if (nm) CK(cudaMemcpyAsync(h_status.data(), sl.status.p, size_t(nm) * 4, cudaMemcpyDeviceToHost, ss));
    CK(cudaStreamSynchronize(ss));
    for (uint32_t i = 0; i < nm; ++i)
        if (h_status[i] != 0) return fail_out(set_err(ctx, VTX_E_INVALID, "vtx_submit_bam: BGZF member %u failed with decoder status %d (corrupt data)", i, h_status[i]));
    if (hs[1] & (stage::kErrWalk | stage::kErrRecord))
        return fail_out(set_err(ctx, VTX_E_INVALID, "vtx_submit_bam: the record walk did not land on the index's record boundaries (corrupt BAM record or index; flags %u)", hs[1]));
    n_rec = hs[0];
    const size_t nrp = size_t(n_rec) + 1;
    ENS(sl.rec_off, nrp * 8); ENS(sl.rec_tid, nrp * 4); ENS(sl.rec_pos, nrp * 4); ENS(sl.rec_end, nrp * 4); ENS(sl.rec_fm, nrp * 4); ENS(sl.used, nrp * 4);
    ENS(sl.cand_count, size_t(nl + 1) * 4); ENS(sl.cand_first, size_t(nl + 2) * 4); ENS(sl.cand_start, size_t(nl + 2) * 8);
    stage::LocusMetrics* d_met = P<stage::LocusMetrics>(ctx->bam_metrics);
    uint64_t n_cand = 0;
    uint32_t max_read = 0;
    if (n_rec) {
        stage::vtx_k_walk<<<blocks_for(n_seg, stage::kWalkWarps), stage::kWalkWarps * 32, 0, ss>>>(sp, n_seg, P<uint64_t>(sl.entry), 1, nullptr, P<uint32_t>(sl.seg_first), P<uint64_t>(sl.rec_off), d_sc + 1);
        stage::vtx_k_parse<<<blocks_for(n_rec, 256), 256, 0, ss>>>(sp, n_rec, P<uint64_t>(sl.rec_off), P<int32_t>(sl.rec_tid), P<int32_t>(sl.rec_pos),
                                                                   P<int32_t>(sl.rec_end), P<uint32_t>(sl.rec_fm), d_sc + 2);
        CK(cudaMemsetAsync(sl.used.p, 0, nrp * 4, ss));
    }
    if (nl) {
        ENS(sl.status, std::max<size_t>(size_t(nm) * 4 + 16, sizeof(stage::LocusMetrics) + 16));
        stage::LocusMetrics* d_tmp = reinterpret_cast<stage::LocusMetrics*>(sl.status.p);
        CK(cudaMemsetAsync(d_tmp, 0, sizeof(stage::LocusMetrics), ss));
        if (ctx->locus_stats) ENS(sl.lfilt, size_t(nl) * stage::kNumCounters * 4);
        stage::vtx_k_locus_cands<<<blocks_for(nl, 64), 64, 0, ss>>>(sp, nl, P<int64_t>(sl.l_start), P<int64_t>(sl.l_end), n_rec, P<uint64_t>(sl.rec_off),
                                                                   P<int32_t>(sl.rec_tid), P<int32_t>(sl.rec_pos), P<int32_t>(sl.rec_end), P<uint32_t>(sl.rec_fm),
                                                                   d_sc + 2, d_sc + 3, 0, P<uint32_t>(sl.cand_count), nullptr, nullptr, nullptr, d_tmp,
                                                                   ctx->locus_stats ? P<uint32_t>(sl.lfilt) : nullptr);
        rc = scan_u32(ctx, ss, ctx->stage_sums, P<uint32_t>(sl.cand_count), nl, P<uint32_t>(sl.cand_first), nullptr);
        if (rc) return fail_out(rc);
        CK(cudaMemcpyAsync(hs, P<uint32_t>(sl.cand_first) + nl, 4, cudaMemcpyDeviceToHost, ss));
    } else hs[0] = 0;
    CK(cudaMemcpyAsync(hs + 1, d_sc + 1, 12, cudaMemcpyDeviceToHost, ss));
    CK(cudaStreamSynchronize(ss));
    n_cand = hs[0]; max_read = hs[3];
    if (hs[1] & (stage::kErrWalk | stage::kErrRecord)) return fail_out(set_err(ctx, VTX_E_INVALID, "vtx_submit_bam: corrupt BAM record (flags %u)", hs[1]));
    if (max_read > uint32_t(kMaxRead)) return fail_out(set_err(ctx, VTX_E_UNSUPPORTED, "reads longer than %d bases (biased int16 DP) are not supported (%u)", kMaxRead, max_read));
    if (n_cand >= 0xFFFFFFF0ull) return fail_out(set_err(ctx, VTX_E_INVALID, "n_cand exceeds 2^32 per shard; split the shard"));
    const size_t ncp = size_t(n_cand) + 1;
    ENS(sl.cand_rec, ncp * 4); ENS(sl.read_off, nrp * 8); ENS(sl.read_len, nrp * 4); ENS(sl.read_cb_off, nrp * 4); ENS(sl.read_cb_len, nrp * 2 + 2);
    if (ctx->cfg.use_umi) ENS(sl.read_umi, nrp * 8);
    if (nl) {
        stage::LocusMetrics* d_tmp = reinterpret_cast<stage::LocusMetrics*>(sl.status.p);
        stage::vtx_k_locus_cands<<<blocks_for(nl, 64), 64, 0, ss>>>(sp, nl, P<int64_t>(sl.l_start), P<int64_t>(sl.l_end), n_rec, P<uint64_t>(sl.rec_off),
                                                                   P<int32_t>(sl.rec_tid), P<int32_t>(sl.rec_pos), P<int32_t>(sl.rec_end), P<uint32_t>(sl.rec_fm),
                                                                   d_sc + 2, d_sc + 3, 1, nullptr, P<uint32_t>(sl.cand_first), P<uint32_t>(sl.cand_rec), P<uint32_t>(sl.used), d_tmp,
                                                                   nullptr);
        stage::vtx_k_widen<<<blocks_for(nl + 1, 256), 256, 0, ss>>>(nl + 1, P<uint32_t>(sl.cand_first), P<uint64_t>(sl.cand_start));
    }
    if (n_rec)
        stage::vtx_k_read_emit<<<blocks_for(n_rec, 128), 128, 0, ss>>>(sp, n_rec, P<uint64_t>(sl.rec_off), P<uint32_t>(sl.used), P<uint64_t>(sl.read_off),
                                                                       P<uint32_t>(sl.read_len), P<uint32_t>(sl.read_cb_off), P<uint16_t>(sl.read_cb_len),
                                                                       P<uint64_t>(sl.read_umi), d_sc + 1);
    if (name_keys && n_rec) {
        uint32_t tab_size = 1;
        while (tab_size < 2 * n_rec) tab_size <<= 1;
        ENS(sl.name_tab, size_t(tab_size) * 4);
        CK(cudaMemsetAsync(sl.name_tab.p, 0xFF, size_t(tab_size) * 4, ss));
        stage::vtx_k_name_key<<<blocks_for(n_rec, 128), 128, 0, ss>>>(sp, n_rec, P<uint64_t>(sl.rec_off), P<uint32_t>(sl.used),
                                                                      P<uint32_t>(sl.name_tab), tab_size - 1, P<uint64_t>(sl.read_umi));
    }
    CK(cudaGetLastError());
    if (ctx->cfg.use_umi && !name_keys && n_rec) {
        CK(cudaMemcpyAsync(hs + 1, d_sc + 1, 4, cudaMemcpyDeviceToHost, ss));
        CK(cudaStreamSynchronize(ss));
        if (hs[1] & stage::kErrExoticUmi) return fail_out(set_err(ctx, VTX_E_UNSUPPORTED, "vtx_submit_bam: a UB tag outside vtx_pack_umi's alphabet needs the host's interner; stage this shard on the host"));
    }
    if (nl) {
        stage::LocusMetrics* d_tmp = reinterpret_cast<stage::LocusMetrics*>(sl.status.p);
        vtx_k_add_u64<<<1, 32, 0, ss>>>(reinterpret_cast<unsigned long long*>(d_met), reinterpret_cast<const unsigned long long*>(d_tmp),
                                        int(sizeof(stage::LocusMetrics) / 8));
    }
    CK(cudaEventRecord(sl.staged, ss));
    DevBatch d{};
    d.n_loci = nl; d.n_reads = n_rec; d.n_cand = n_cand;
    d.locus_row = P<uint32_t>(sl.locus_row); d.hap = P<uint8_t>(sl.hap); d.ref_off = P<uint32_t>(sl.ref_off); d.ref_len = P<uint32_t>(sl.ref_len);
    d.alt_off = P<uint32_t>(sl.alt_off); d.alt_len = P<uint32_t>(sl.alt_len); d.cand_start = P<uint64_t>(sl.cand_start);
    d.read_nib = P<uint8_t>(sl.stream); d.read_off = P<uint64_t>(sl.read_off); d.read_len = P<uint32_t>(sl.read_len);
    d.cb_bytes = P<uint8_t>(sl.stream); d.read_cb_off = P<uint32_t>(sl.read_cb_off); d.read_cb_len = P<uint16_t>(sl.read_cb_len);
    d.read_umi = ctx->cfg.use_umi ? P<uint64_t>(sl.read_umi) : nullptr; d.cand_read = P<uint32_t>(sl.cand_rec);
    d.max_read_len = max_read; d.max_hap_len = max_hap;
    d.lfilt = ctx->locus_stats && nl ? P<uint32_t>(sl.lfilt) : nullptr;
    CK(cudaStreamWaitEvent(ctx->stream, sl.staged, 0));
    CK(cudaEventRecord(tr->ev[EV_C0], ctx->stream));
    rc = process_batch(ctx, d, tr);
    if (rc) return rc;
    CK(cudaEventRecord(sl.free_ev, ctx->stream));
    return VTX_OK;
}

int vtx_bam_metrics_get(vtx_ctx* ctx, vtx_bam_metrics* out)
{
    if (!ctx || !out) return VTX_E_INVALID;
    memset(out, 0, sizeof(*out));
    if (!ctx->stage_stream) return VTX_OK;
    CK(cudaSetDevice(ctx->device));
    static_assert(sizeof(vtx_bam_metrics) == offsetof(stage::LocusMetrics, num_low_base_quality) &&
                  offsetof(stage::LocusMetrics, num_low_base_quality) == stage::kLowBaseQuality * sizeof(unsigned long long),
                  "metric layouts must agree");
    CK(cudaMemcpyAsync(out, ctx->bam_metrics.p, sizeof(*out), cudaMemcpyDeviceToHost, ctx->stage_stream));
    CK(cudaStreamSynchronize(ctx->stage_stream));
    return VTX_OK;
}

int vtx_set_min_base_quality(vtx_ctx* ctx, uint32_t min_q)
{
    if (!ctx) return VTX_E_INVALID;
    if (min_q > stage::kMaxBaseQuality) return set_err(ctx, VTX_E_INVALID, "min base quality %u out of range (0..%u)", min_q, stage::kMaxBaseQuality);
    ctx->min_base_quality = min_q;
    return VTX_OK;
}

int vtx_bam_low_base_quality(vtx_ctx* ctx, uint64_t* out)
{
    if (!ctx || !out) return VTX_E_INVALID;
    *out = 0;
    if (!ctx->stage_stream) return VTX_OK;
    CK(cudaSetDevice(ctx->device));
    CK(cudaMemcpyAsync(out, static_cast<const uint8_t*>(ctx->bam_metrics.p) + offsetof(stage::LocusMetrics, num_low_base_quality), 8,
                       cudaMemcpyDeviceToHost, ctx->stage_stream));
    CK(cudaStreamSynchronize(ctx->stage_stream));
    return VTX_OK;
}

int vtx_set_locus_stats(vtx_ctx* ctx, int32_t on)
{
    if (!ctx) return VTX_E_INVALID;
    if (ctx->submitted) return set_err(ctx, VTX_E_STATE, "vtx_set_locus_stats must be called before the first submit");
    ctx->locus_stats = on != 0;
    return VTX_OK;
}

int vtx_locus_stats_get(vtx_ctx* ctx, const vtx_locus_stats** out, uint64_t* n)
{
    if (!ctx || !out || !n) return VTX_E_INVALID;
    *out = nullptr; *n = 0;
    if (!ctx->locus_stats) return set_err(ctx, VTX_E_STATE, "locus statistics are off: call vtx_set_locus_stats(ctx, 1) before the first submit");
    if (!ctx->finished) return set_err(ctx, VTX_E_STATE, "vtx_locus_stats_get must follow vtx_finish / vtx_finish_device");
    *out = ctx->stats_last_n ? ctx->h_lstats.as<const vtx_locus_stats>() : nullptr;
    *n = ctx->stats_last_n;
    return VTX_OK;
}

int vtx_set_donors(vtx_ctx* ctx, uint32_t n_donors, uint64_t n_rows, const uint8_t* dosage, double error_rate)
{
    using namespace donors;
    if (!ctx) return VTX_E_INVALID;
    if (ctx->submitted) return set_err(ctx, VTX_E_STATE, "vtx_set_donors must be called before the first submit");
    if (n_donors < kMinDonors || n_donors > kMaxDonors)
        return set_err(ctx, VTX_E_INVALID, "vtx_set_donors: %u donors; 2 to 32 are supported", n_donors);
    if (!(error_rate >= 1e-6 && error_rate <= 0.25))
        return set_err(ctx, VTX_E_INVALID, "vtx_set_donors: error rate %g outside [1e-6, 0.25]", error_rate);
    if (n_rows && !dosage) return set_err(ctx, VTX_E_INVALID, "vtx_set_donors: dosage is NULL");
    const size_t cells = size_t(n_rows) * n_donors;
    std::vector<uint8_t> usable(size_t(n_rows) + 1, 0);
    for (size_t i = 0; i < cells; ++i)
        if (dosage[i] > 2 && dosage[i] != kMissing)
            return set_err(ctx, VTX_E_INVALID, "vtx_set_donors: dosage %u at row %zu, donor %zu (0, 1, 2 or VTX_GT_MISSING)",
                           unsigned(dosage[i]), i / n_donors, i % n_donors);
    for (uint64_t r = 0; r < n_rows; ++r) usable[r] = row_usable(dosage + size_t(r) * n_donors, n_donors) ? 1 : 0;
    CK(cudaSetDevice(ctx->device));
    ENS(ctx->donor_dosage, cells + 16);
    ENS(ctx->donor_usable, usable.size());
    if (cells) CK(cudaMemcpy(ctx->donor_dosage.p, dosage, cells, cudaMemcpyHostToDevice));
    CK(cudaMemcpy(ctx->donor_usable.p, usable.data(), usable.size(), cudaMemcpyHostToDevice));
    ctx->n_donors = n_donors;
    ctx->donor_rows = n_rows;
    ctx->donor_tab = make_tables(error_rate);
    ctx->donors = true;
    ctx->donor_valid = false;
    return VTX_OK;
}

int vtx_donor_ll_get(vtx_ctx* ctx, const int64_t** ll, const uint64_t** counts, uint32_t* n_cols, uint32_t* n_hyp)
{
    if (!ctx || !ll || !counts || !n_cols || !n_hyp) return VTX_E_INVALID;
    *ll = nullptr; *counts = nullptr; *n_cols = 0; *n_hyp = 0;
    if (!ctx->donors) return set_err(ctx, VTX_E_STATE, "no donors: call vtx_set_donors before the first submit");
    if (!ctx->finished || !ctx->donor_valid) return set_err(ctx, VTX_E_STATE, "vtx_donor_ll_get must follow vtx_finish / vtx_finish_device");
    const uint32_t H = donors::n_hyp(ctx->n_donors);
    *ll = ctx->h_donor.as<const int64_t>();
    *counts = reinterpret_cast<const uint64_t*>(*ll + size_t(ctx->donor_last_cols) * H);
    *n_cols = ctx->donor_last_cols;
    *n_hyp = H;
    return VTX_OK;
}

uint64_t vtx_pack_cb(const uint8_t* s, uint32_t len) { return (s || len == 0) ? stage::pack_cb(s, len) : VTX_NO_CB_KEY; }

int vtx_sync(vtx_ctx* ctx)
{
    if (!ctx) return VTX_E_INVALID;
    CK(cudaSetDevice(ctx->device));
    CK(cudaStreamSynchronize(ctx->stream));
    return VTX_OK;
}

int vtx_wait_copies(vtx_ctx* ctx)
{
    if (!ctx) return VTX_E_INVALID;
    CK(cudaSetDevice(ctx->device));
    CK(cudaStreamSynchronize(ctx->copy_stream));
    return VTX_OK;
}

static int finish_scalars(vtx_ctx* ctx)
{
    CK(cudaSetDevice(ctx->device));
    uint64_t* hs = ctx->h_scalars.as<uint64_t>();
    CK(cudaMemcpyAsync(hs, ctx->d_res_n.p, 8, cudaMemcpyDeviceToHost, ctx->stream));
    CK(cudaMemcpyAsync(hs + 1, ctx->d_metrics.p, 48, cudaMemcpyDeviceToHost, ctx->stream));
    const uint64_t sn = ctx->finished ? 0 : ctx->stats_n;
    if (sn) {
        if (sn > ctx->h_lstats_cap) {
            const size_t ncap = size_t(sn) + size_t(sn) / 4 + 1024;
            const cudaError_t e = ctx->h_lstats.alloc(ncap * sizeof(vtx_locus_stats));
            if (e != cudaSuccess) { ctx->h_lstats_cap = 0; return set_err(ctx, VTX_E_NOMEM, "pinned locus statistics alloc failed: %s", cudaGetErrorString(e)); }
            ctx->h_lstats_cap = ncap;
        }
        CK(cudaMemcpyAsync(ctx->h_lstats.p, ctx->lstats.p, size_t(sn) * sizeof(vtx_locus_stats), cudaMemcpyDeviceToHost, ctx->stream));
    }
    uint64_t donor_bad = 0;
    if (ctx->donors) {
        const uint32_t cols = ctx->finished ? ctx->n_barcodes : ctx->donor_cols;
        const size_t bytes = donor_acc_bytes(cols, donors::n_hyp(ctx->n_donors));
        if (bytes > ctx->h_donor_cap) {
            ctx->donor_valid = false;
            const cudaError_t e = ctx->h_donor.alloc(bytes);
            if (e != cudaSuccess) { ctx->h_donor_cap = 0; return set_err(ctx, VTX_E_NOMEM, "pinned donor log-likelihood alloc failed: %s", cudaGetErrorString(e)); }
            ctx->h_donor_cap = bytes;
        }
        if (ctx->finished) memset(ctx->h_donor.p, 0, bytes);
        else CK(cudaMemcpyAsync(ctx->h_donor.p, ctx->donor_acc.p, bytes, cudaMemcpyDeviceToHost, ctx->stream));
        CK(cudaStreamSynchronize(ctx->stream));
        memcpy(&donor_bad, ctx->h_donor.as<uint8_t>() + bytes - 8, 8);
        ctx->donor_last_cols = cols;
        ctx->donor_valid = true;
    }
    CK(cudaStreamSynchronize(ctx->stream));
    ctx->stats_last_n = sn;
    ctx->stats_n = 0;
    const uint64_t violated = ctx->finished ? 0 : hs[5], band_overflow = ctx->finished ? 0 : hs[6];
    ctx->last_n = ctx->finished ? 0 : hs[0];
    ctx->last_metrics.num_not_cell_bc = ctx->finished ? 0 : hs[1];
    ctx->last_metrics.num_non_umi = ctx->finished ? 0 : hs[2];
    ctx->last_metrics.num_scored = ctx->finished ? 0 : hs[3];
    ctx->t_pairs = ctx->last_metrics.num_scored;
    ctx->finished = true;
    if (band_overflow)
        return set_err(ctx, VTX_E_UNSUPPORTED, "band model: %llu alignments had more k-mer hits than the work buffers hold (reads x windows too large); "
                                               "they were scored with the full matrix", (unsigned long long)band_overflow);
    if (donor_bad)
        return set_err(ctx, VTX_E_INVALID, "%llu loci have a row outside the donor dosage table given to vtx_set_donors (%llu rows); "
                                           "they were left out of the donor log-likelihoods", (unsigned long long)donor_bad,
                       (unsigned long long)ctx->donor_rows);
    if (violated)
        return set_err(ctx, VTX_E_INVALID, "%llu loci of a device batch exceeded the bounds given to vtx_submit_device(_ex) (longest read / widest "
                                           "haplotype window); they were skipped, the result is incomplete", (unsigned long long)violated);
    return VTX_OK;
}

int vtx_finish_device(vtx_ctx* ctx, vtx_result* out)
{
    Nvtx nvtx_range("vtx_finish_device");
    if (!ctx || !out) return VTX_E_INVALID;
    int rc = finish_scalars(ctx);
    if (rc) return rc;
    point_result(out, ptrs(ctx->res), 0x7Fu, ctx->last_n, ctx->last_metrics);
    return VTX_OK;
}

int vtx_fetch(vtx_ctx* ctx, const vtx_result* device_result, vtx_result* out)
{
    Nvtx nvtx_range("vtx_fetch");
    if (!ctx || !device_result || !out) return VTX_E_INVALID;
    CK(cudaSetDevice(ctx->device));
    const bool gathered = device_result->row == ctx->g_dev[0].p && ctx->g_dev[0].p != nullptr;
    HostResults& h = gathered ? ctx->g_host : ctx->h_res;
    const vtx_result& dev = *device_result;
    const size_t n = dev.n;
    int rc = ensure_host(ctx, h, n);
    if (rc) return rc;
    if (n) {
        rc = copy_results(ctx, h, { dev.row, dev.col, dev.ref_cnt, dev.alt_cnt, dev.unk_cnt, dev.val, dev.val2 }, 0, n, ctx->stream);
        if (rc) return rc;
        CK(cudaStreamSynchronize(ctx->stream));
    }
    point_result(out, ptrs(h.a), want_mask(ctx), n, dev.metrics);
    return VTX_OK;
}

int vtx_finish(vtx_ctx* ctx, vtx_result* out)
{
    Nvtx nvtx_range("vtx_finish");
    if (!ctx || !out) return VTX_E_INVALID;
    CK(cudaSetDevice(ctx->device));
    const auto src = ptrs(ctx->res);
    size_t fetched = 0;
    const bool streamed = !ctx->finished && ctx->h_cum.p && ctx->fetch_stream && ctx->trec_used > 0 && ctx->trec_used <= kMaxCum;
    if (streamed) {
        int rc = ensure_host(ctx, ctx->h_res, ctx->res_ub);
        if (rc) return rc;
        for (size_t i = 0; i < ctx->trec_used; ++i) {
            CK(cudaEventSynchronize(ctx->trecs[i].ev[EV_POST]));
            const size_t n_i = size_t(ctx->h_cum.as<unsigned long long>()[i]);
            if (n_i > fetched && n_i <= ctx->h_res.cap) {
                rc = copy_results(ctx, ctx->h_res, src, fetched, n_i, ctx->fetch_stream);
                if (rc) return rc;
                fetched = n_i;
            }
        }
    }
    vtx_result dev{};
    int rc = vtx_finish_device(ctx, &dev);
    if (rc) return rc;
    const size_t n = dev.n;
    rc = ensure_host(ctx, ctx->h_res, n);
    if (rc) return rc;
    cudaStream_t st = ctx->fetch_stream ? ctx->fetch_stream : ctx->stream;
    if (n > fetched) {
        rc = copy_results(ctx, ctx->h_res, src, fetched, n, st);
        if (rc) return rc;
    }
    CK(cudaStreamSynchronize(st));
    point_result(out, ptrs(ctx->h_res.a), want_mask(ctx), n, dev.metrics);
    return VTX_OK;
}
int vtx_last_tile_counts(vtx_ctx* ctx, uint32_t* out, uint32_t n_out)
{
    if (!ctx || !out) return VTX_E_INVALID;
    if (!ctx->last_tiles_valid) return set_err(ctx, VTX_E_STATE, "no Smith-Waterman pass has run yet");
    CK(cudaSetDevice(ctx->device));
    CK(cudaStreamSynchronize(ctx->stream));
    const uint32_t nl = ctx->last_tiles_nl;
    for (uint32_t c = 0; c < n_out; ++c) {
        out[c] = 0;
        if (c < uint32_t(kNumClasses))
            CK(cudaMemcpy(out + c, P<uint32_t>(ctx->tstart) + size_t(c) * (nl + 1) + nl, 4, cudaMemcpyDeviceToHost));
    }
    return kNumClasses;
}

int vtx_last_timing(vtx_ctx* ctx, vtx_timing* t)
{
    if (!ctx || !t) return VTX_E_INVALID;
    if (!ctx->timing_valid || ctx->trec_used == 0) return set_err(ctx, VTX_E_STATE, "no finished submit to time");
    CK(cudaSetDevice(ctx->device));
    memset(t, 0, sizeof(*t));
    for (size_t i = 0; i < ctx->trec_used; ++i) {
        TimeRec& r = ctx->trecs[i];
        CK(cudaEventSynchronize(r.ev[EV_POST]));
        float ms = 0;
        if (r.had_h2d) { CK(cudaEventElapsedTime(&ms, r.ev[EV_START], r.ev[EV_H2D])); t->h2d_ms += ms; }
        CK(cudaEventElapsedTime(&ms, r.ev[EV_C0], r.ev[EV_PREP])); t->prep_ms += ms;
        CK(cudaEventElapsedTime(&ms, r.ev[EV_PREP], r.ev[EV_SW])); t->sw_ms += ms;
        CK(cudaEventElapsedTime(&ms, r.ev[EV_SW], r.ev[EV_POST])); t->post_ms += ms;
        t->sw_launches += r.sw_launches; t->total_launches += r.launches;
    }
    t->n_pairs = ctx->t_pairs;
    return VTX_OK;
}

int vtx_score_pairs(vtx_ctx* ctx, const vtx_batch* hb, uint64_t n_pairs, const uint32_t* pair_read,
                    const uint32_t* pair_locus, int16_t* ref_score, int16_t* alt_score)
{
    Nvtx nvtx_range("vtx_score_pairs");
    if (!ctx) return VTX_E_INVALID;
    if (!hb) return set_err(ctx, VTX_E_INVALID, "batch is NULL");
    BatchView hv0 = view_of(hb); hv0.n_cand = 0; hv0.cand_read = nullptr;
    int rc = validate_batch(ctx, hv0);
    if (rc) return rc;
    if (n_pairs >= 0xFFFFFFF0ull) return set_err(ctx, VTX_E_INVALID, "too many pairs");
    if (n_pairs && (!pair_read || !pair_locus || !ref_score || !alt_score)) return set_err(ctx, VTX_E_INVALID, "NULL pair arrays");
    DevBatch d{};
    rc = scan_host_batch(ctx, hv0, &d.max_read_len, &d.max_hap_len, false);
    if (rc) return rc;
    if (n_pairs == 0) return VTX_OK;
    const uint32_t nl = hb->n_loci;
    std::vector<uint32_t> start(size_t(nl) + 2, 0), order(n_pairs), s_read(n_pairs), s_locus(n_pairs);
    for (uint64_t i = 0; i < n_pairs; ++i) {
        if (pair_locus[i] >= nl || pair_read[i] >= hb->n_reads) return set_err(ctx, VTX_E_INVALID, "pair %llu out of range", (unsigned long long)i);
        ++start[pair_locus[i] + 1];
    }
    for (uint32_t l = 0; l < nl; ++l) start[l + 1] += start[l];
    {
        std::vector<uint32_t> cur(start.begin(), start.begin() + nl + 1);
        for (uint64_t i = 0; i < n_pairs; ++i) { const uint32_t p = cur[pair_locus[i]]++; order[p] = uint32_t(i); s_read[p] = pair_read[i]; s_locus[p] = pair_locus[i]; }
    }
    CK(cudaSetDevice(ctx->device));
    InSlot* sl = nullptr;
    rc = claim_slot(ctx, &sl);
    if (rc) return rc;
    rc = upload_common(ctx, sl, hv0, d);
    if (rc) return rc;
    CK(cudaEventRecord(sl->copy_done, ctx->copy_stream));
    CK(cudaStreamWaitEvent(ctx->stream, sl->copy_done, 0));
    ENS(ctx->pair_read, n_pairs * 4 + 4); ENS(ctx->pair_locus, n_pairs * 4 + 4); ENS(ctx->pair_start, size_t(nl + 1) * 4);
    ENS(ctx->pair_scores, n_pairs * 4 + 4);
    CK(cudaMemcpyAsync(ctx->pair_read.p, s_read.data(), n_pairs * 4, cudaMemcpyHostToDevice, ctx->stream));
    CK(cudaMemcpyAsync(ctx->pair_locus.p, s_locus.data(), n_pairs * 4, cudaMemcpyHostToDevice, ctx->stream));
    vtx_k_pair_start_explicit<<<blocks_for(nl + 1, 256), 256, 0, ctx->stream>>>(nl, uint32_t(n_pairs), P<uint32_t>(ctx->pair_locus),
                                                                                P<uint32_t>(ctx->pair_start));
    uint64_t launches = 1, sw_launches = 0;
    rc = run_sw(ctx, d, uint32_t(n_pairs), nullptr, nullptr, P<uint32_t>(ctx->pair_scores), &launches, &sw_launches, nullptr);
    if (rc) return rc;
    CK(cudaEventRecord(sl->free_ev, ctx->stream));
    std::vector<uint32_t> packed(n_pairs);
    CK(cudaMemcpyAsync(packed.data(), ctx->pair_scores.p, n_pairs * 4, cudaMemcpyDeviceToHost, ctx->stream));
    CK(cudaStreamSynchronize(ctx->stream));
    for (uint64_t p = 0; p < n_pairs; ++p) {
        ref_score[order[p]] = int16_t(packed[p] & 0xFFFF);
        alt_score[order[p]] = int16_t(packed[p] >> 16);
    }
    return VTX_OK;
}

uint64_t vtx_pack_umi(const uint8_t* s, uint32_t len) { return stage::pack_umi(s, len); }


}

#include <dlfcn.h>
namespace {
typedef struct { char internal[128]; } nccl_uid;
typedef void* nccl_comm;
struct NcclApi {
    void* h = nullptr;
    int (*GetUniqueId)(nccl_uid*) = nullptr;
    int (*CommInitRank)(nccl_comm*, int, nccl_uid, int) = nullptr;
    int (*CommDestroy)(nccl_comm) = nullptr;
    int (*AllGather)(const void*, void*, size_t, int, nccl_comm, cudaStream_t) = nullptr;
    int (*Broadcast)(const void*, void*, size_t, int, int, nccl_comm, cudaStream_t) = nullptr;
    int (*Send)(const void*, size_t, int, int, nccl_comm, cudaStream_t) = nullptr;
    int (*Recv)(void*, size_t, int, int, nccl_comm, cudaStream_t) = nullptr;
    int (*GroupStart)() = nullptr;
    int (*GroupEnd)() = nullptr;
    const char* (*GetErrorString)(int) = nullptr;
    bool ok = false;
};
NcclApi g_nccl;
constexpr int kNcclUint8 = 1, kNcclUint64 = 5;

bool load_nccl(std::string* why)
{
    if (g_nccl.ok) return true;
    const char* names[] = { "libnccl.so.2", "libnccl.so" };
    for (const char* n : names) { g_nccl.h = dlopen(n, RTLD_NOW | RTLD_GLOBAL); if (g_nccl.h) break; }
    if (!g_nccl.h) { *why = std::string("dlopen(libnccl.so.2) failed: ") + dlerror(); return false; }
#define SYM(field, name) *(void**)(&g_nccl.field) = dlsym(g_nccl.h, name); if (!g_nccl.field) { *why = std::string("missing symbol ") + name; return false; }
    SYM(GetUniqueId, "ncclGetUniqueId") SYM(CommInitRank, "ncclCommInitRank") SYM(CommDestroy, "ncclCommDestroy")
    SYM(AllGather, "ncclAllGather") SYM(Broadcast, "ncclBroadcast") SYM(GroupStart, "ncclGroupStart")
    SYM(GroupEnd, "ncclGroupEnd") SYM(GetErrorString, "ncclGetErrorString") SYM(Send, "ncclSend") SYM(Recv, "ncclRecv")
#undef SYM
    g_nccl.ok = true;
    return true;
}
#define NK(call) do { int r_ = (call); if (r_ != 0) return set_err(ctx, VTX_E_NCCL, "%s failed: %s", #call, g_nccl.GetErrorString(r_)); } while (0)

void comm_destroy(vtx_ctx* ctx)
{
    if (ctx->comm && g_nccl.ok) g_nccl.CommDestroy(static_cast<nccl_comm>(ctx->comm));
    ctx->comm = nullptr;
}
}

extern "C" {

int vtx_comm_unique_id(uint8_t id_out[128])
{
    std::string why;
    if (!id_out) return VTX_E_INVALID;
    if (!load_nccl(&why)) { g_create_error = why; return VTX_E_NCCL; }
    nccl_uid id;
    int r = g_nccl.GetUniqueId(&id);
    if (r != 0) { g_create_error = g_nccl.GetErrorString(r); return VTX_E_NCCL; }
    memcpy(id_out, id.internal, 128);
    return VTX_OK;
}

int vtx_comm_init(vtx_ctx* ctx, const uint8_t id[128], int32_t rank, int32_t n_ranks)
{
    if (!ctx || !id || n_ranks < 1 || rank < 0 || rank >= n_ranks) return ctx ? set_err(ctx, VTX_E_INVALID, "vtx_comm_init: bad arguments") : VTX_E_INVALID;
    std::string why;
    if (!load_nccl(&why)) return set_err(ctx, VTX_E_NCCL, "%s", why.c_str());
    CK(cudaSetDevice(ctx->device));
    nccl_uid uid; memcpy(uid.internal, id, 128);
    nccl_comm comm = nullptr;
    NK(g_nccl.CommInitRank(&comm, n_ranks, uid, rank));
    ctx->comm = comm; ctx->rank = rank; ctx->n_ranks = n_ranks;
    return VTX_OK;
}

int vtx_gather_start(vtx_ctx* ctx, int32_t root)
{
    Nvtx nvtx_range("vtx_gather_start");
    if (!ctx) return VTX_E_INVALID;
    if (!ctx->finished) return set_err(ctx, VTX_E_STATE, "vtx_gather must follow vtx_finish / vtx_finish_device");
    if (ctx->gather_pending) return set_err(ctx, VTX_E_STATE, "a gather is already in flight: call vtx_gather_wait first");
    const int nrk = ctx->n_ranks;
    if (root != VTX_GATHER_ALL && (root < 0 || root >= nrk)) return set_err(ctx, VTX_E_INVALID, "gather root %d out of range", root);
    if (nrk != 1 && !ctx->comm) return set_err(ctx, VTX_E_STATE, "vtx_comm_init has not been called");
    CK(cudaSetDevice(ctx->device));
    const uint32_t want = want_mask(ctx);
    const DBuf* loc = ctx->res;
    vtx_result& out = ctx->g_out;
    if (nrk == 1) {
        point_result(&out, ptrs(ctx->res), want, ctx->last_n, ctx->last_metrics);
    } else {
        if (!ctx->comm_stream) {
            CK(cudaStreamCreateWithFlags(&ctx->comm_stream, cudaStreamNonBlocking));
            CK(cudaEventCreateWithFlags(&ctx->ev_counts, cudaEventDisableTiming));
            CK(cudaEventCreateWithFlags(&ctx->ev_gather, cudaEventDisableTiming));
            CK(cudaEventCreateWithFlags(&ctx->ev_results, cudaEventDisableTiming));
            CK(ctx->h_counts.alloc(size_t(nrk + 1) * 32));
        }
        cudaStream_t cs = ctx->comm_stream;
        nccl_comm comm = static_cast<nccl_comm>(ctx->comm);
        CK(cudaEventRecord(ctx->ev_results, ctx->stream));
        CK(cudaStreamWaitEvent(cs, ctx->ev_results, 0));
        ENS(ctx->g_counts, size_t(nrk + 1) * 32);
        uint64_t* mine = ctx->h_counts.as<uint64_t>() + size_t(nrk) * 4;
        mine[0] = ctx->last_n; mine[1] = ctx->last_metrics.num_not_cell_bc; mine[2] = ctx->last_metrics.num_non_umi; mine[3] = ctx->last_metrics.num_scored;
        uint64_t* dmine = P<uint64_t>(ctx->g_counts) + size_t(nrk) * 4;
        CK(cudaMemcpyAsync(dmine, mine, 32, cudaMemcpyHostToDevice, cs));
        NK(g_nccl.AllGather(dmine, ctx->g_counts.p, 4, kNcclUint64, comm, cs));
        CK(cudaMemcpyAsync(ctx->h_counts.p, ctx->g_counts.p, size_t(nrk) * 32, cudaMemcpyDeviceToHost, cs));
        CK(cudaEventRecord(ctx->ev_counts, cs));
        CK(cudaEventSynchronize(ctx->ev_counts));
        const uint64_t* counts = ctx->h_counts.as<uint64_t>();
        size_t total = 0;
        std::vector<size_t> offs(nrk);
        vtx_metrics met{};
        for (int r = 0; r < nrk; ++r) {
            offs[r] = total; total += counts[size_t(r) * 4];
            met.num_not_cell_bc += counts[size_t(r) * 4 + 1]; met.num_non_umi += counts[size_t(r) * 4 + 2]; met.num_scored += counts[size_t(r) * 4 + 3];
        }
        const bool receiver = root == VTX_GATHER_ALL || root == ctx->rank;
        if (receiver) for (int i = 0; i < kResArrays; ++i) if (want >> i & 1) ENS(ctx->g_dev[i], (total ? total : 1) * kResEsz[i]);
        NK(g_nccl.GroupStart());
        for (int i = 0; i < kResArrays; ++i) {
            if (!(want >> i & 1)) continue;
            const size_t esz = kResEsz[i];
            if (root == VTX_GATHER_ALL) {
                for (int r = 0; r < nrk; ++r) {
                    const size_t n = counts[size_t(r) * 4];
                    if (n) NK(g_nccl.Broadcast(loc[i].p, static_cast<uint8_t*>(ctx->g_dev[i].p) + offs[r] * esz, n * esz, kNcclUint8, r, comm, cs));
                }
            } else if (ctx->rank == root) {
                for (int r = 0; r < nrk; ++r) {
                    const size_t n = counts[size_t(r) * 4];
                    if (!n) continue;
                    uint8_t* dst = static_cast<uint8_t*>(ctx->g_dev[i].p) + offs[r] * esz;
                    if (r == root) CK(cudaMemcpyAsync(dst, loc[i].p, n * esz, cudaMemcpyDeviceToDevice, cs));
                    else NK(g_nccl.Recv(dst, n * esz, kNcclUint8, r, comm, cs));
                }
            } else if (ctx->last_n) {
                NK(g_nccl.Send(loc[i].p, size_t(ctx->last_n) * esz, kNcclUint8, root, comm, cs));
            }
        }
        NK(g_nccl.GroupEnd());
        CK(cudaEventRecord(ctx->ev_gather, cs));
        ctx->gather_guard = true;
        point_result(&out, ptrs(ctx->g_dev), receiver ? want : 0u, total, met);
    }
    ctx->gather_pending = true;
    return VTX_OK;
}

int vtx_gather_wait(vtx_ctx* ctx, vtx_result* out)
{
    Nvtx nvtx_range("vtx_gather_wait");
    if (!ctx || !out) return VTX_E_INVALID;
    if (!ctx->gather_pending) return set_err(ctx, VTX_E_STATE, "no gather in flight");
    CK(cudaSetDevice(ctx->device));
    if (ctx->n_ranks > 1) CK(cudaEventSynchronize(ctx->ev_gather));
    ctx->gather_pending = false;
    *out = ctx->g_out;
    return VTX_OK;
}

int vtx_gather(vtx_ctx* ctx, vtx_result* out)
{
    if (!ctx || !out) return VTX_E_INVALID;
    const int rc = vtx_gather_start(ctx, VTX_GATHER_ALL);
    return rc ? rc : vtx_gather_wait(ctx, out);
}

}
```

vartrix_b200/csrc/vtx_pipeline.cuh:

```cuda
#pragma once
#include <cstdint>
#include <cuda_runtime.h>
#include "vtx_sw.cuh"
#include "vtx_sw_split.cuh"
#include "vtx_sw_fold.cuh"
#include "vtx_record.cuh"

namespace vtx {

constexpr uint32_t kNoCb = 0xFFFFFFFFu;
constexpr uint64_t kNoUmi = 0xFFFFFFFFFFFFFFFFull;
constexpr uint32_t kInvalid = 0xFFFFFFFFu;

__host__ __device__ inline uint64_t fnv1a64(const uint8_t* p, uint32_t n)
{
    uint64_t h = 1469598103934665603ull;
    for (uint32_t i = 0; i < n; ++i) { h ^= p[i]; h *= 1099511628211ull; }
    return h;
}

struct BarcodeTable {
    const int32_t* slot;
    uint32_t cap_mask;
    const uint8_t* bytes;
    const uint32_t* off;
};

__device__ __forceinline__ int32_t cb_lookup_bytes(const BarcodeTable& t, const uint8_t* __restrict__ key, uint32_t len)
{
    uint32_t h = uint32_t(fnv1a64(key, len)) & t.cap_mask;
    for (;;) {
        const int32_t s = t.slot[h];
        if (s < 0) return -1;
        const uint32_t o = t.off[s], l2 = t.off[s + 1] - o;
        if (l2 == len) {
            bool eq = true;
            for (uint32_t i = 0; i < len; ++i) eq &= (t.bytes[o + i] == key[i]);
            if (eq) return s;
        }
        h = (h + 1) & t.cap_mask;
    }
}

__global__ void vtx_k_cb_lookup(BarcodeTable t, uint32_t n_reads, const uint8_t* __restrict__ cb_bytes,
                                const uint32_t* __restrict__ read_cb_off, const uint16_t* __restrict__ read_cb_len,
                                int32_t* __restrict__ read_col)
{
    const uint32_t r = blockIdx.x * blockDim.x + threadIdx.x;
    if (r >= n_reads) return;
    const uint32_t off = read_cb_off[r];
    read_col[r] = off != kNoCb ? cb_lookup_bytes(t, cb_bytes + off, read_cb_len[r]) : -1;
}

using stage::kNoCbKey;
constexpr uint64_t kCbExotic = 0x8000000000000000ull;

__host__ __device__ inline uint64_t mix64(uint64_t x)
{
    x ^= x >> 30; x *= 0xbf58476d1ce4e5b9ull; x ^= x >> 27; x *= 0x94d049bb133111ebull; x ^= x >> 31;
    return x;
}

struct BarcodeKeyTable {
    const uint64_t* key;
    const uint32_t* idx;
    uint32_t cap_mask;
};

__global__ void vtx_k_cb_lookup_key(BarcodeTable t, BarcodeKeyTable kt, uint32_t n_reads, const uint64_t* __restrict__ read_cb_key,
                                    const uint8_t* __restrict__ cb_bytes, const uint32_t* __restrict__ cb_off,
                                    int32_t* __restrict__ read_col)
{
    const uint32_t r = blockIdx.x * blockDim.x + threadIdx.x;
    if (r >= n_reads) return;
    const uint64_t key = read_cb_key[r];
    int32_t col = -1;
    if (key == kNoCbKey) {
    } else if (key & kCbExotic) {
        const uint32_t i = uint32_t(key & 0xFFFFFFFFu);
        col = cb_lookup_bytes(t, cb_bytes + cb_off[i], cb_off[i + 1] - cb_off[i]);
    } else {
        uint32_t h = uint32_t(mix64(key)) & kt.cap_mask;
        for (;;) {
            const uint64_t k = kt.key[h];
            if (k == key) { col = int32_t(kt.idx[h]); break; }
            if (k == kNoCbKey) break;
            h = (h + 1) & kt.cap_mask;
        }
    }
    read_col[r] = col;
}

__global__ void vtx_k_read_units(uint32_t n_reads, const uint16_t* __restrict__ read_len, uint32_t* __restrict__ units)
{
    const uint32_t r = blockIdx.x * blockDim.x + threadIdx.x;
    if (r < n_reads) units[r] = ((uint32_t(read_len[r]) + 1) / 2 + 3) / 4;
}
__global__ void vtx_k_expand_reads(uint32_t n_reads, const uint16_t* __restrict__ read_len, const uint32_t* __restrict__ off4,
                                   uint64_t* __restrict__ read_off, uint32_t* __restrict__ read_len32)
{
    const uint32_t r = blockIdx.x * blockDim.x + threadIdx.x;
    if (r >= n_reads) return;
    read_off[r] = uint64_t(off4[r]) * 4;
    read_len32[r] = read_len[r];
}

__global__ void vtx_k_cand_filter(uint64_t n_cand, const uint32_t* __restrict__ cand_read,
                                  const int32_t* __restrict__ read_col, const uint64_t* __restrict__ read_umi_key,
                                  int use_umi, uint32_t* __restrict__ keep, unsigned long long* __restrict__ metrics)
{
    const uint64_t c = uint64_t(blockIdx.x) * blockDim.x + threadIdx.x;
    bool miss_cb = false, miss_umi = false, ok = false;
    if (c < n_cand) {
        const uint32_t r = cand_read ? cand_read[c] : uint32_t(c);
        if (read_col[r] < 0) miss_cb = true;
        else if (use_umi && read_umi_key[r] == kNoUmi) miss_umi = true;
        else ok = true;
        keep[c] = ok ? 1u : 0u;
    }
    __shared__ uint32_t s_cnt[3];
    if (threadIdx.x < 3) s_cnt[threadIdx.x] = 0;
    __syncthreads();
    const uint32_t b0 = __ballot_sync(0xffffffffu, miss_cb), b1 = __ballot_sync(0xffffffffu, miss_umi),
                   b2 = __ballot_sync(0xffffffffu, ok);
    if ((threadIdx.x & 31) == 0) {
        if (b0) atomicAdd(&s_cnt[0], uint32_t(__popc(b0)));
        if (b1) atomicAdd(&s_cnt[1], uint32_t(__popc(b1)));
        if (b2) atomicAdd(&s_cnt[2], uint32_t(__popc(b2)));
    }
    __syncthreads();
    if (threadIdx.x < 3 && s_cnt[threadIdx.x]) atomicAdd(metrics + threadIdx.x, (unsigned long long)s_cnt[threadIdx.x]);
}

__device__ __forceinline__ uint32_t locus_of_cand(const uint64_t* __restrict__ cand_start, uint32_t n_loci, uint64_t c)
{
    uint32_t lo = 0, hi = n_loci;
    while (hi - lo > 1) {
        const uint32_t mid = (lo + hi) >> 1;
        if (cand_start[mid] <= c) lo = mid; else hi = mid;
    }
    return lo;
}

__global__ void vtx_k_compact(uint64_t n_cand, const uint32_t* __restrict__ cand_read,
                              const uint32_t* __restrict__ keep, const uint32_t* __restrict__ pidx,
                              const int32_t* __restrict__ read_col, const uint64_t* __restrict__ read_umi_key,
                              int use_umi, uint32_t* __restrict__ pair_read, uint32_t* __restrict__ pair_col,
                              uint64_t* __restrict__ pair_umi)
{
    const uint64_t c = uint64_t(blockIdx.x) * blockDim.x + threadIdx.x;
    if (c >= n_cand || !keep[c]) return;
    const uint32_t p = pidx[c], r = cand_read ? cand_read[c] : uint32_t(c);
    pair_read[p] = r;
    pair_col[p] = uint32_t(read_col[r]);
    if (use_umi) pair_umi[p] = read_umi_key[r];
}

__global__ void vtx_k_pair_start(uint32_t n_loci, const uint64_t* __restrict__ cand_start,
                                 const uint32_t* __restrict__ pidx, uint32_t* __restrict__ pair_start)
{
    const uint32_t l = blockIdx.x * blockDim.x + threadIdx.x;
    if (l <= n_loci) pair_start[l] = pidx[cand_start[l]];
}

__global__ void vtx_k_pair_start_explicit(uint32_t n_loci, uint32_t n_pairs, const uint32_t* __restrict__ pair_locus,
                                          uint32_t* __restrict__ pair_start)
{
    const uint32_t l = blockIdx.x * blockDim.x + threadIdx.x;
    if (l > n_loci) return;
    uint32_t lo = 0, hi = n_pairs;
    while (lo < hi) { const uint32_t mid = (lo + hi) >> 1; if (pair_locus[mid] < l) lo = mid + 1; else hi = mid; }
    pair_start[l] = lo;
}

__global__ void vtx_k_locus_prep(uint32_t n_loci, const uint8_t* __restrict__ hap_bytes,
                                 const uint32_t* __restrict__ ref_off, const uint32_t* __restrict__ ref_len,
                                 const uint32_t* __restrict__ alt_off, const uint32_t* __restrict__ alt_len,
                                 const uint32_t* __restrict__ pair_start, const uint32_t* __restrict__ pair_read,
                                 const uint32_t* __restrict__ read_len, SwAllow allow,
                                 uint32_t max_read, uint32_t max_hap, unsigned long long* __restrict__ bounds_violated,
                                 uint32_t* __restrict__ tcount )
{
    const uint32_t l = (blockIdx.x * blockDim.x + threadIdx.x) >> 5;
    const int lane = threadIdx.x & 31;
    if (l >= n_loci) return;
    const uint32_t nr = ref_len[l], na = alt_len[l];
    const uint8_t* rh = hap_bytes + ref_off[l];
    const uint8_t* ah = hap_bytes + alt_off[l];
    LocusShape s;
    bool exotic = false;
    for (uint32_t j = lane; j < nr; j += 32) exotic |= is_exotic(rh[j]);
    for (uint32_t j = lane; j < na; j += 32) exotic |= is_exotic(ah[j]);
    s.exotic = __any_sync(0xffffffffu, exotic);
    bool same = prefix_possible(nr, na);
    if (same) for (uint32_t j = lane; j < uint32_t(kSplitP); j += 32) same &= (rh[j] == ah[j]);
    s.prefix = __all_sync(0xffffffffu, same);
    bool fold = s.prefix && allow.fold && fold_possible(nr, na);
    if (fold) for (uint32_t j = lane; j < uint32_t(kFoldP); j += 32) fold &= (rh[nr - 1 - j] == ah[na - 1 - j]);
    s.fold = __all_sync(0xffffffffu, fold);
    uint32_t longest = 0;
    for (uint32_t p = pair_start[l] + lane; p < pair_start[l + 1]; p += 32) longest = max(longest, read_len[pair_read[p]]);
    longest = __reduce_max_sync(0xffffffffu, longest);
    if (lane != 0) return;
    s.width = max(nr, na);
    if (longest > max_read || s.width > max_hap) {
        atomicAdd(bounds_violated, 1ull);
#pragma unroll
        for (int c = 0; c < kNumClasses; ++c) tcount[size_t(c) * (n_loci + 1) + l] = 0u;
        return;
    }
    const int cls = tile_class(s, allow, longest);
    const uint32_t np = pair_start[l + 1] - pair_start[l];
#pragma unroll
    for (int c = 0; c < kNumClasses; ++c)
        tcount[size_t(c) * (n_loci + 1) + l] = (c == cls) ? (np + pairs_per_tile(c) - 1) / pairs_per_tile(c) : 0u;
}

constexpr int kSlotThreads = 128;
constexpr int kSlotChunk = 1024;
constexpr uint32_t kSlotSmallMax = 2048;
constexpr int kSlotBigThreads = 1024;
constexpr int kSlotBigWords = 7;
__global__ void __launch_bounds__(kSlotThreads) vtx_k_slots(
    uint32_t n_loci, const uint32_t* __restrict__ pair_start, const uint32_t* __restrict__ pair_col,
    const uint64_t* __restrict__ pair_umi, int use_umi, uint8_t* __restrict__ pair_first,
    uint32_t* __restrict__ pair_cslot, uint32_t* __restrict__ pair_uslot, uint32_t* __restrict__ cslot_col,
    uint32_t* __restrict__ cslot_locus, uint32_t* __restrict__ uslot_cslot, uint32_t* __restrict__ big_list )
{
    __shared__ uint32_t s_col[kSlotChunk];
    __shared__ uint64_t s_umi[kSlotChunk];
    __shared__ uint8_t s_first[kSlotChunk];
    for (uint32_t l = blockIdx.x; l < n_loci; l += gridDim.x) {
        const uint32_t ps = pair_start[l], d = pair_start[l + 1] - ps;
        if (d == 0) continue;
        if (d > kSlotSmallMax) {
            if (threadIdx.x == 0) big_list[1 + atomicAdd(big_list, 1u)] = l;
            continue;
        }
        for (uint32_t base = 0; base < d; base += kSlotThreads) {
            const uint32_t p = base + threadIdx.x;
            uint32_t colp = 0; uint64_t umip = 0; bool fc = true, fu = true;
            if (p < d) { colp = pair_col[ps + p]; if (use_umi) umip = pair_umi[ps + p]; }
            const uint32_t q_end = min(d, base + kSlotThreads);
            for (uint32_t q0 = 0; q0 < q_end; q0 += kSlotChunk) {
                __syncthreads();
                for (uint32_t i = threadIdx.x; i < kSlotChunk && q0 + i < q_end; i += kSlotThreads) {
                    s_col[i] = pair_col[ps + q0 + i];
                    if (use_umi) s_umi[i] = pair_umi[ps + q0 + i];
                }
                __syncthreads();
                if (p < d) {
                    const uint32_t lim = min(uint32_t(kSlotChunk), min(q_end, p) > q0 ? min(q_end, p) - q0 : 0u);
                    for (uint32_t i = 0; i < lim; ++i) {
                        if (s_col[i] == colp) { fc = false; if (!use_umi || s_umi[i] == umip) fu = false; }
                    }
                }
            }
            if (p < d) pair_first[ps + p] = uint8_t((fc ? 1 : 0) | (fu ? 2 : 0));
        }
        __syncthreads();
        for (uint32_t base = 0; base < d; base += kSlotThreads) {
            const uint32_t p = base + threadIdx.x;
            uint32_t colp = 0; uint64_t umip = 0; uint32_t cs = 0, us = 0;
            if (p < d) { colp = pair_col[ps + p]; if (use_umi) umip = pair_umi[ps + p]; }
            for (uint32_t q0 = 0; q0 < d; q0 += kSlotChunk) {
                __syncthreads();
                for (uint32_t i = threadIdx.x; i < kSlotChunk && q0 + i < d; i += kSlotThreads) {
                    s_col[i] = pair_col[ps + q0 + i];
                    s_first[i] = pair_first[ps + q0 + i];
                    if (use_umi) s_umi[i] = pair_umi[ps + q0 + i];
                }
                __syncthreads();
                if (p < d) {
                    const uint32_t lim = min(uint32_t(kSlotChunk), d - q0);
                    for (uint32_t i = 0; i < lim; ++i) {
                        const uint32_t cq = s_col[i]; const uint8_t fq = s_first[i];
                        cs += ((fq & 1) && cq < colp) ? 1u : 0u;
                        if (use_umi) us += ((fq & 2) && (cq < colp || (cq == colp && s_umi[i] < umip))) ? 1u : 0u;
                    }
                }
            }
            if (p < d) {
                const uint8_t fp = pair_first[ps + p];
                pair_cslot[ps + p] = ps + cs;
                if (fp & 1) { cslot_col[ps + cs] = colp; cslot_locus[ps + cs] = l; }
                if (use_umi) {
                    pair_uslot[ps + p] = ps + us;
                    if (fp & 2) uslot_cslot[ps + us] = ps + cs;
                }
            }
        }
        __syncthreads();
    }
}

__device__ __forceinline__ uint32_t mix32(uint32_t x) { x ^= x >> 16; x *= 0x7feb352du; x ^= x >> 15; x *= 0x846ca68bu; x ^= x >> 16; return x; }

__global__ void __launch_bounds__(kSlotBigThreads) vtx_k_slots_big(
    const uint32_t* __restrict__ big_list, const uint32_t* __restrict__ pair_start, const uint32_t* __restrict__ pair_col,
    const uint64_t* __restrict__ pair_umi, int use_umi, uint32_t* __restrict__ scratch, uint32_t* __restrict__ pair_cslot,
    uint32_t* __restrict__ pair_uslot, uint32_t* __restrict__ cslot_col, uint32_t* __restrict__ cslot_locus,
    uint32_t* __restrict__ uslot_cslot)
{
    __shared__ uint32_t s_count;
    const uint32_t n_big = big_list[0];
    const uint32_t tid = threadIdx.x;
    for (uint32_t bi = blockIdx.x; bi < n_big; bi += gridDim.x) {
        const uint32_t l = big_list[1 + bi];
        const uint32_t ps = pair_start[l], d = pair_start[l + 1] - ps;
        const uint32_t cap = 2 * d;
        uint32_t* ctab = scratch + size_t(kSlotBigWords) * ps;
        uint32_t* dcols = ctab + cap;
        uint32_t* utab = dcols + d;
        uint32_t* uid = utab + cap;
        for (uint32_t i = tid; i < cap; i += kSlotBigThreads) { ctab[i] = kInvalid; if (use_umi) utab[i] = kInvalid; }
        if (tid == 0) s_count = 0;
        __syncthreads();
        for (uint32_t p = tid; p < d; p += kSlotBigThreads) {
            const uint32_t col = pair_col[ps + p];
            uint32_t h = mix32(col) % cap;
            for (;;) {
                const uint32_t old = atomicCAS(&ctab[h], kInvalid, col);
                if (old == kInvalid || old == col) break;
                h = h + 1 == cap ? 0 : h + 1;
            }
        }
        __syncthreads();
        for (uint32_t i = tid; i < cap; i += kSlotBigThreads)
            if (ctab[i] != kInvalid) dcols[atomicAdd(&s_count, 1u)] = ctab[i];
        __syncthreads();
        const uint32_t D = s_count;
        uint32_t P = 1;
        while (P < D) P <<= 1;
        __syncthreads();
        for (uint32_t i = tid; i < P; i += kSlotBigThreads) ctab[i] = i < D ? dcols[i] : kInvalid;
        __syncthreads();
        for (uint32_t k = 2; k <= P; k <<= 1)
            for (uint32_t j = k >> 1; j > 0; j >>= 1) {
                for (uint32_t i = tid; i < P; i += kSlotBigThreads) {
                    const uint32_t q = i ^ j;
                    if (q > i) {
                        const uint32_t a = ctab[i], b = ctab[q];
                        const bool up = (i & k) == 0;
                        if ((a > b) == up) { ctab[i] = b; ctab[q] = a; }
                    }
                }
                __syncthreads();
            }
        for (uint32_t p = tid; p < d; p += kSlotBigThreads) {
            const uint32_t col = pair_col[ps + p];
            uint32_t lo = 0, hi = D;
            while (lo < hi) { const uint32_t mid = (lo + hi) >> 1; if (ctab[mid] < col) lo = mid + 1; else hi = mid; }
            pair_cslot[ps + p] = ps + lo;
            cslot_col[ps + lo] = col;
            cslot_locus[ps + lo] = l;
        }
        if (use_umi) {
            if (tid == 0) s_count = 0;
            __syncthreads();
            for (uint32_t p = tid; p < d; p += kSlotBigThreads) {
                const uint32_t col = pair_col[ps + p]; const uint64_t umi = pair_umi[ps + p];
                uint32_t h = mix32(col ^ mix32(uint32_t(umi) ^ mix32(uint32_t(umi >> 32)))) % cap;
                for (;;) {
                    uint32_t cur = utab[h];
                    if (cur == kInvalid) { cur = atomicCAS(&utab[h], kInvalid, p); if (cur == kInvalid) break; }
                    if (pair_col[ps + cur] == col && pair_umi[ps + cur] == umi) break;
                    h = h + 1 == cap ? 0 : h + 1;
                }
            }
            __syncthreads();
            for (uint32_t i = tid; i < cap; i += kSlotBigThreads)
                if (utab[i] != kInvalid) uid[i] = atomicAdd(&s_count, 1u);
            __syncthreads();
            for (uint32_t p = tid; p < d; p += kSlotBigThreads) {
                const uint32_t col = pair_col[ps + p]; const uint64_t umi = pair_umi[ps + p];
                uint32_t h = mix32(col ^ mix32(uint32_t(umi) ^ mix32(uint32_t(umi >> 32)))) % cap;
                for (;;) {
                    const uint32_t cur = utab[h];
                    if (pair_col[ps + cur] == col && pair_umi[ps + cur] == umi) break;
                    h = h + 1 == cap ? 0 : h + 1;
                }
                const uint32_t us = ps + uid[h];
                pair_uslot[ps + p] = us;
                uslot_cslot[us] = pair_cslot[ps + p];
            }
        }
        __syncthreads();
    }
}

__global__ void vtx_k_umi_collapse(uint32_t n_slots_ub, const uint32_t* __restrict__ n_pairs_ptr,
                                   const uint32_t* __restrict__ uslot_cslot, const uint32_t* __restrict__ ucnt,
                                   uint32_t* __restrict__ ccnt)
{
    const uint32_t q = blockIdx.x * blockDim.x + threadIdx.x;
    if (q >= n_slots_ub || q >= *n_pairs_ptr) return;
    const uint32_t cs = uslot_cslot[q];
    if (cs == kInvalid) return;
    const uint4 c = reinterpret_cast<const uint4*>(ucnt)[q];
    const uint32_t r = c.x, a = c.y, u = c.z, t = r + a + u;
    if (t == 0) return;
    uint32_t k;
    if (4ull * a >= 3ull * t) k = 1;
    else if (4ull * r >= 3ull * t) k = 0;
    else k = 2;
    atomicAdd(ccnt + size_t(cs) * 4 + k, 1u);
}

__global__ void vtx_k_finalize(uint32_t n_slots_ub, const uint32_t* __restrict__ n_pairs_ptr, int mode,
                               const uint32_t* __restrict__ cslot_col, const uint32_t* __restrict__ ccnt,
                               uint32_t* __restrict__ keep)
{
    const uint32_t q = blockIdx.x * blockDim.x + threadIdx.x;
    if (q >= n_slots_ub) return;
    uint32_t k = 0;
    if (q < *n_pairs_ptr && cslot_col[q] != kInvalid) {
        if (mode == 0) {
            const uint4 c = reinterpret_cast<const uint4*>(ccnt)[q];
            k = (c.x > 0 || c.y > 0) ? 1u : 0u;
        } else k = 1u;
    }
    keep[q] = k;
}

struct ResultArrays {
    uint32_t* row; uint32_t* col; uint32_t* ref_cnt; uint32_t* alt_cnt; uint32_t* unk_cnt;
    double* val; double* val2;
};

__global__ void vtx_k_emit(uint32_t n_slots_ub, int mode, const uint32_t* __restrict__ keep,
                           const uint32_t* __restrict__ oidx, const unsigned long long* __restrict__ res_base,
                           const uint32_t* __restrict__ cslot_col, const uint32_t* __restrict__ cslot_locus,
                           const uint32_t* __restrict__ locus_row, const uint32_t* __restrict__ ccnt, ResultArrays out)
{
    const uint32_t q = blockIdx.x * blockDim.x + threadIdx.x;
    if (q >= n_slots_ub || !keep[q]) return;
    const uint64_t o = *res_base + oidx[q];
    const uint4 c = reinterpret_cast<const uint4*>(ccnt)[q];
    const uint32_t r = c.x, a = c.y, u = c.z;
    out.row[o] = locus_row[cslot_locus[q]];
    out.col[o] = cslot_col[q];
    out.ref_cnt[o] = r; out.alt_cnt[o] = a; out.unk_cnt[o] = u;
    double v = 0.0, v2 = 0.0;
    if (mode == 0) v = (r > 0 && a > 0) ? 3.0 : (a > 0 ? 2.0 : 1.0);
    else if (mode == 2) v = double(a) / (double(r) + double(a) + double(u));
    else { v = double(a); v2 = double(r); }
    out.val[o] = v; out.val2[o] = v2;
}

__global__ void vtx_k_add_u64(unsigned long long* dst, const unsigned long long* __restrict__ src, int n)
{
    if (blockIdx.x == 0 && int(threadIdx.x) < n) dst[threadIdx.x] += src[threadIdx.x];
}

__global__ void vtx_k_bump(unsigned long long* res_n, const uint32_t* __restrict__ total, unsigned long long* cum_host)
{
    if (threadIdx.x == 0 && blockIdx.x == 0) {
        const unsigned long long n = *res_n + (total ? *total : 0u);
        *res_n = n;
        if (cum_host) *cum_host = n;
    }
}

constexpr int kScanThreads = 256;
constexpr int kScanItems = 8;
constexpr int kScanTile = kScanThreads * kScanItems;

__device__ __forceinline__ uint32_t block_exclusive_scan(uint32_t v, uint32_t* total)
{
    __shared__ uint32_t warp_sums[kScanThreads / 32];
    __shared__ uint32_t s_total;
    const int lane = threadIdx.x & 31, w = threadIdx.x >> 5;
    uint32_t x = v;
#pragma unroll
    for (int o = 1; o < 32; o <<= 1) { const uint32_t y = __shfl_up_sync(0xffffffffu, x, o); if (lane >= o) x += y; }
    if (lane == 31) warp_sums[w] = x;
    __syncthreads();
    if (w == 0) {
        uint32_t s = lane < kScanThreads / 32 ? warp_sums[lane] : 0;
#pragma unroll
        for (int o = 1; o < 32; o <<= 1) { const uint32_t y = __shfl_up_sync(0xffffffffu, s, o); if (lane >= o) s += y; }
        if (lane < kScanThreads / 32) warp_sums[lane] = s;
        if (lane == kScanThreads / 32 - 1) s_total = s;
    }
    __syncthreads();
    const uint32_t prefix = (w ? warp_sums[w - 1] : 0) + x - v;
    *total = s_total;
    __syncthreads();
    return prefix;
}

__global__ void __launch_bounds__(kScanThreads) vtx_k_scan_tiles(const uint32_t* __restrict__ in, uint64_t n,
                                                                 uint32_t* __restrict__ out, uint32_t* __restrict__ sums)
{
    const uint64_t base = uint64_t(blockIdx.x) * kScanTile + uint64_t(threadIdx.x) * kScanItems;
    uint32_t v[kScanItems], s = 0;
#pragma unroll
    for (int i = 0; i < kScanItems; ++i) { v[i] = (base + i < n) ? in[base + i] : 0; s += v[i]; }
    uint32_t total;
    uint32_t p = block_exclusive_scan(s, &total);
#pragma unroll
    for (int i = 0; i < kScanItems; ++i) { if (base + i < n) out[base + i] = p; p += v[i]; }
    if (threadIdx.x == 0) sums[blockIdx.x] = total;
}

__global__ void __launch_bounds__(kScanThreads) vtx_k_scan_sums(uint32_t* __restrict__ sums, uint32_t n_blocks,
                                                                uint32_t* __restrict__ total_out)
{
    uint32_t carry = 0;
    for (uint32_t base = 0; base < n_blocks; base += kScanThreads) {
        const uint32_t i = base + threadIdx.x;
        const uint32_t v = i < n_blocks ? sums[i] : 0;
        uint32_t total;
        const uint32_t p = block_exclusive_scan(v, &total);
        if (i < n_blocks) sums[i] = carry + p;
        carry += total;
    }
    if (threadIdx.x == 0) *total_out = carry;
}

__global__ void __launch_bounds__(kScanThreads) vtx_k_scan_rows(const uint32_t* __restrict__ in, uint32_t* __restrict__ out,
                                                                uint32_t n, uint32_t stride)
{
    const uint32_t* src = in + size_t(blockIdx.x) * stride;
    uint32_t* dst = out + size_t(blockIdx.x) * stride;
    uint32_t carry = 0;
    for (uint32_t base = 0; base < n; base += kScanTile) {
        const uint32_t i0 = base + threadIdx.x * kScanItems;
        uint32_t v[kScanItems], sum = 0;
#pragma unroll
        for (int k = 0; k < kScanItems; ++k) { v[k] = (i0 + k < n) ? src[i0 + k] : 0; sum += v[k]; }
        uint32_t total;
        uint32_t p = carry + block_exclusive_scan(sum, &total);
#pragma unroll
        for (int k = 0; k < kScanItems; ++k) { if (i0 + k < n) dst[i0 + k] = p; p += v[k]; }
        carry += total;
    }
    if (threadIdx.x == 0) dst[n] = carry;
}

__global__ void __launch_bounds__(kScanThreads) vtx_k_scan_add(uint32_t* __restrict__ out, uint64_t n,
                                                               const uint32_t* __restrict__ sums)
{
    const uint64_t base = uint64_t(blockIdx.x) * kScanTile + uint64_t(threadIdx.x) * kScanItems;
    const uint32_t add = sums[blockIdx.x];
#pragma unroll
    for (int i = 0; i < kScanItems; ++i) if (base + i < n) out[base + i] += add;
}

}
```

Before: 177.0 million.

## Replace three-pass scans with single-pass decoupled lookback and fuse filter/compact/emit kernels

Introduces a single-pass decoupled-lookback scan, with a tile ticket and per-tile state that is memset before each use. It uses this to fuse candidate filtering, scanning and compaction into one kernel, finalize, scan and emit into another, and read-unit computation with offset expansion into a third. The per-class row scan also moves onto the lookback kernel. SW occupancy queries are now cached per kernel and smem size. This cuts kernel launches and intermediate keep/index buffers in the prep and post stages, at the cost of inter-block spin-waiting and extra memsets.

```diff
diff --git a/vartrix_b200/csrc/vtx_api.cu b/vartrix_b200/csrc/vtx_api.cu
--- a/vartrix_b200/csrc/vtx_api.cu
+++ b/vartrix_b200/csrc/vtx_api.cu
@@ -15,8 +15,10 @@
 #include <cstddef>
 #include <cstdio>
 #include <cstring>
+#include <map>
 #include <string>
 #include <thread>
+#include <utility>
 #include <vector>
 
 using namespace vtx;
@@ -111,10 +113,11 @@
     DBuf bc_slot, bc_bytes, bc_off;
     DBuf bck_key, bck_idx;
     uint32_t bck_cap = 0;
-    DBuf x_read_off, x_read_len, x_units, x_off4;
+    DBuf x_read_off, x_read_len;
     DBuf band_scratch;
     DBuf inf_comp, inf_out, inf_desc, inf_status;
     bool inflate_attr_set = false;
+    std::map<std::pair<const void*, size_t>, int> sw_per_sm;
     StageSlot sslot[2];
     uint64_t n_bam_submits = 0;
     cudaStream_t stage_stream = nullptr;
@@ -142,8 +145,8 @@
     InSlot slot[2];
     uint64_t n_submits = 0;
     cudaStream_t copy_stream = nullptr;
-    DBuf read_col, keep, pidx, scan_sums, pair_read, pair_col, pair_umi, pair_locus, pair_start, tcount, tstart,
-        pair_first, pair_cslot, pair_uslot, cslot_col, cslot_locus, uslot_cslot, ccnt, ucnt, keep2, oidx, tile_counters,
+    DBuf read_col, pidx, scan_sums, pair_read, pair_col, pair_umi, pair_locus, pair_start, tcount, tstart,
+        pair_first, pair_cslot, pair_uslot, cslot_col, cslot_locus, uslot_cslot, ccnt, ucnt, tile_counters,
         scratch, pair_scores, d_metrics, d_res_n, big_list, slot_scratch;
     DBuf res[kResArrays];
     size_t res_cap = 0;
@@ -228,14 +231,37 @@
 
 inline unsigned blocks_for(uint64_t n, unsigned threads) { return unsigned((n + threads - 1) / threads); }
 
+int lookback_state(vtx_ctx* ctx, cudaStream_t st, DBuf& buf, uint64_t tiles, uint32_t rows, Lookback* lb)
+{
+    const size_t bytes = lookback_bytes(tiles, rows);
+    ENS(buf, bytes);
+    CK(cudaMemsetAsync(buf.p, 0, bytes, st));
+    lb->state = P<unsigned long long>(buf);
+    return VTX_OK;
+}
+
+inline unsigned scan_tiles(uint64_t n) { return std::max(1u, blocks_for(n, kScanTile)); }
+
 int scan_u32(vtx_ctx* ctx, cudaStream_t st, DBuf& sums, const uint32_t* in, uint64_t n, uint32_t* out, uint64_t* launches)
 {
-    const unsigned nb = std::max(1u, blocks_for(n, kScanTile));
+    const unsigned nb = scan_tiles(n);
+    Lookback lb;
+    int rc = lookback_state(ctx, st, sums, nb, 1, &lb);
+    if (rc) return rc;
+    vtx_k_scan<<<nb, kScanThreads, 0, st>>>(in, n, n, out, lb);
+    if (launches) ++*launches;
+    CK(cudaGetLastError());
+    return VTX_OK;
+}
+
+int scan_u32_three_pass(vtx_ctx* ctx, cudaStream_t st, DBuf& sums, const uint32_t* in, uint64_t n, uint32_t* out, uint64_t* launches)
+{
+    const unsigned nb = scan_tiles(n);
     ENS(sums, size_t(nb) * 4);
     vtx_k_scan_tiles<<<nb, kScanThreads, 0, st>>>(in, n, out, P<uint32_t>(sums));
     vtx_k_scan_sums<<<1, kScanThreads, 0, st>>>(P<uint32_t>(sums), nb, out + n);
     vtx_k_scan_add<<<nb, kScanThreads, 0, st>>>(out, n, P<uint32_t>(sums));
-    if (launches) *launches += 3;
+    *launches += 3;
     CK(cudaGetLastError());
     return VTX_OK;
 }
@@ -321,8 +347,14 @@
               const char* name, int cls)
 {
     CK(cudaFuncSetAttribute(kern, cudaFuncAttributeMaxDynamicSharedMemorySize, int(smem)));
-    int per_sm = 0;
-    CK(cudaOccupancyMaxActiveBlocksPerMultiprocessor(&per_sm, kern, threads, smem));
+    const auto key = std::make_pair(reinterpret_cast<const void*>(kern), smem);
+    auto it = ctx->sw_per_sm.find(key);
+    if (it == ctx->sw_per_sm.end()) {
+        int n = 0;
+        CK(cudaOccupancyMaxActiveBlocksPerMultiprocessor(&n, kern, threads, smem));
+        it = ctx->sw_per_sm.emplace(key, n).first;
+    }
+    const int per_sm = it->second;
     if (per_sm < 1) {
         if (cls < 0) return set_err(ctx, VTX_E_CUDA, "%s does not fit on an SM (smem %zu)", name, smem);
         return set_err(ctx, VTX_E_CUDA, "%s %d does not fit on an SM (smem %zu)", name, cls, smem);
@@ -362,7 +394,11 @@
         nl, b.hap, b.ref_off, b.ref_len, b.alt_off, b.alt_len, P<uint32_t>(ctx->pair_start), P<uint32_t>(ctx->pair_read), b.read_len,
         allow, b.max_read_len, b.max_hap_len, P<unsigned long long>(ctx->d_metrics) + 4, P<uint32_t>(ctx->tcount));
     ++*launches;
-    vtx_k_scan_rows<<<kNumClasses, kScanThreads, 0, ctx->stream>>>(P<uint32_t>(ctx->tcount), P<uint32_t>(ctx->tstart), nl, nl + 1);
+    Lookback lb;
+    int rc = lookback_state(ctx, ctx->stream, ctx->scan_sums, scan_tiles(nl), kNumClasses, &lb);
+    if (rc) return rc;
+    vtx_k_scan<<<dim3(scan_tiles(nl), kNumClasses), kScanThreads, 0, ctx->stream>>>(P<uint32_t>(ctx->tcount), nl, nl + 1,
+                                                                                    P<uint32_t>(ctx->tstart), lb);
     ++*launches;
     CK(cudaGetLastError());
     CK(cudaMemsetAsync(ctx->tile_counters.p, 0, 64, ctx->stream));
@@ -413,7 +449,7 @@
         if (!(mask >> c & 1u)) continue;
         a.tile_start = P<uint32_t>(ctx->tstart) + size_t(c) * (nl + 1);
         a.tile_counter = P<uint32_t>(ctx->tile_counters) + c;
-        int rc = VTX_OK;
+        rc = VTX_OK;
         switch (c) {
         case 0: rc = launch_sw_class<0>(ctx, a, launches); break;
         case 1: rc = launch_sw_class<1>(ctx, a, launches); break;
@@ -523,7 +559,7 @@
     if (!n_slots) return VTX_OK;
     ENS(ctx->donor_start, (size_t(nc) + 1) * 4);
     ENS(ctx->donor_list, size_t(n_slots_ub) * 4 + 4);
-    int rc = scan_u32(ctx, st, ctx->scan_sums, P<uint32_t>(ctx->donor_count), nc, P<uint32_t>(ctx->donor_start), launches);
+    int rc = scan_u32_three_pass(ctx, st, ctx->scan_sums, P<uint32_t>(ctx->donor_count), nc, P<uint32_t>(ctx->donor_start), launches);
     if (rc) return rc;
     CK(cudaMemsetAsync(ctx->donor_count.p, 0, size_t(nc) * 4, st));
     vtx_k_donor_scatter<<<grid, kDonorThreads, 0, st>>>(in, n_slots_ub, n_slots, P<uint32_t>(ctx->donor_start),
@@ -570,7 +606,7 @@
 
     const size_t ncp = size_t(nc) + 1;
     ENS(ctx->read_col, size_t(nr ? nr : 1) * 4);
-    ENS(ctx->keep, ncp * 4); ENS(ctx->pidx, ncp * 4);
+    ENS(ctx->pidx, ncp * 4);
     ENS(ctx->pair_read, ncp * 4); ENS(ctx->pair_col, ncp * 4);
     if (use_umi) ENS(ctx->pair_umi, ncp * 8);
     ENS(ctx->pair_start, size_t(nl + 1) * 4);
@@ -578,13 +614,12 @@
     ENS(ctx->pair_cslot, ncp * 4); ENS(ctx->cslot_col, ncp * 4); ENS(ctx->cslot_locus, ncp * 4);
     ENS(ctx->ccnt, ncp * 16);
     if (use_umi) { ENS(ctx->pair_uslot, ncp * 4); ENS(ctx->uslot_cslot, ncp * 4); ENS(ctx->ucnt, ncp * 16); }
-    ENS(ctx->keep2, ncp * 4); ENS(ctx->oidx, ncp * 4);
     uint32_t* pair_scores = nullptr;
     if (ctx->cfg.flags & VTX_F_KEEP_SCORES) { ENS(ctx->pair_scores, ncp * 4); pair_scores = P<uint32_t>(ctx->pair_scores); }
 
     if (nl == 0 || nc == 0) {
         if (ctx->d_cum && ctx->trec_used - 1 < kMaxCum)
-            vtx_k_bump<<<1, 32, 0, st>>>(P<unsigned long long>(ctx->d_res_n), nullptr, ctx->d_cum + (ctx->trec_used - 1));
+            vtx_k_bump<<<1, 32, 0, st>>>(P<unsigned long long>(ctx->d_res_n), ctx->d_cum + (ctx->trec_used - 1));
         CK(cudaEventRecord(tr->ev[EV_PREP], st)); CK(cudaEventRecord(tr->ev[EV_SW], st));
         if (stats) {
             if ((rc = launch_locus_stats(ctx, b, false, &launches))) return rc;
@@ -607,14 +642,13 @@
     } else {
         vtx_k_cb_lookup<<<blocks_for(nr, 256), 256, 0, st>>>(tab, nr, b.cb_bytes, b.read_cb_off, b.read_cb_len, P<int32_t>(ctx->read_col));
     }
-    vtx_k_cand_filter<<<blocks_for(nc, 256), 256, 0, st>>>(nc, b.cand_read, P<int32_t>(ctx->read_col), b.read_umi, use_umi,
-                                                           P<uint32_t>(ctx->keep), P<unsigned long long>(ctx->d_metrics));
-    launches += 2;
-    rc = scan_u32(ctx, st, ctx->scan_sums, P<uint32_t>(ctx->keep), nc, P<uint32_t>(ctx->pidx), &launches);
-    if (rc) return rc;
-    vtx_k_compact<<<blocks_for(nc, 256), 256, 0, st>>>(nc, b.cand_read, P<uint32_t>(ctx->keep), P<uint32_t>(ctx->pidx),
-                                                       P<int32_t>(ctx->read_col), b.read_umi, use_umi, P<uint32_t>(ctx->pair_read),
-                                                       P<uint32_t>(ctx->pair_col), P<uint64_t>(ctx->pair_umi));
+    launches += 1;
+    const unsigned nb = scan_tiles(nc);
+    Lookback lb;
+    if ((rc = lookback_state(ctx, st, ctx->scan_sums, nb, 1, &lb))) return rc;
+    vtx_k_cand_compact<<<nb, kScanThreads, 0, st>>>(nc, b.cand_read, P<int32_t>(ctx->read_col), b.read_umi, use_umi, lb,
+                                                    P<uint32_t>(ctx->pidx), P<uint32_t>(ctx->pair_read), P<uint32_t>(ctx->pair_col),
+                                                    P<uint64_t>(ctx->pair_umi), P<unsigned long long>(ctx->d_metrics));
     vtx_k_pair_start<<<blocks_for(nl + 1, 256), 256, 0, st>>>(nl, b.cand_start, P<uint32_t>(ctx->pidx), P<uint32_t>(ctx->pair_start));
     launches += 2;
     const uint32_t* n_pairs_ptr = P<uint32_t>(ctx->pidx) + nc;
@@ -656,24 +690,19 @@
     }
     if (stats && (rc = launch_locus_stats(ctx, b, true, &launches))) return rc;
     if (donor && (rc = launch_donors(ctx, b, uint32_t(nc), n_pairs_ptr, &launches))) return rc;
-    vtx_k_finalize<<<blocks_for(nc, 256), 256, 0, st>>>(uint32_t(nc), n_pairs_ptr, ctx->cfg.mode, P<uint32_t>(ctx->cslot_col),
-                                                        P<uint32_t>(ctx->ccnt), P<uint32_t>(ctx->keep2));
-    ++launches;
-    rc = scan_u32(ctx, st, ctx->scan_sums, P<uint32_t>(ctx->keep2), nc, P<uint32_t>(ctx->oidx), &launches);
-    if (rc) return rc;
+    if ((rc = lookback_state(ctx, st, ctx->scan_sums, nb, 1, &lb))) return rc;
     if (ctx->gather_guard) {
         CK(cudaStreamWaitEvent(st, ctx->ev_gather, 0));
         ctx->gather_guard = false;
     }
     ResultArrays out{ P<uint32_t>(ctx->res[0]), P<uint32_t>(ctx->res[1]), P<uint32_t>(ctx->res[2]), P<uint32_t>(ctx->res[3]),
                       P<uint32_t>(ctx->res[4]), P<double>(ctx->res[5]), P<double>(ctx->res[6]) };
-    vtx_k_emit<<<blocks_for(nc, 256), 256, 0, st>>>(uint32_t(nc), ctx->cfg.mode, P<uint32_t>(ctx->keep2), P<uint32_t>(ctx->oidx),
-                                                    P<unsigned long long>(ctx->d_res_n), P<uint32_t>(ctx->cslot_col),
-                                                    P<uint32_t>(ctx->cslot_locus), b.locus_row, P<uint32_t>(ctx->ccnt), out);
     const size_t sub_idx = ctx->trec_used - 1;
-    vtx_k_bump<<<1, 32, 0, st>>>(P<unsigned long long>(ctx->d_res_n), P<uint32_t>(ctx->oidx) + nc,
-                                 (ctx->d_cum && sub_idx < kMaxCum) ? ctx->d_cum + sub_idx : nullptr);
-    launches += 2;
+    vtx_k_finalize_emit<<<nb, kScanThreads, 0, st>>>(uint32_t(nc), n_pairs_ptr, ctx->cfg.mode, P<uint32_t>(ctx->cslot_col),
+                                                     P<uint32_t>(ctx->cslot_locus), b.locus_row, P<uint32_t>(ctx->ccnt), lb,
+                                                     P<unsigned long long>(ctx->d_res_n),
+                                                     (ctx->d_cum && sub_idx < kMaxCum) ? ctx->d_cum + sub_idx : nullptr, out);
+    ++launches;
     CK(cudaGetLastError());
     CK(cudaEventRecord(tr->ev[EV_POST], st));
     ctx->res_ub += nc;
@@ -923,13 +952,14 @@
     ENS(ctx->x_read_off, size_t(nr ? nr : 1) * 8); ENS(ctx->x_read_len, size_t(nr ? nr : 1) * 4);
     if (nr) {
         if (!d_off4) {
-            ENS(ctx->x_units, size_t(nr) * 4); ENS(ctx->x_off4, size_t(nr + 1) * 4);
-            vtx_k_read_units<<<blocks_for(nr, 256), 256, 0, ctx->stream>>>(nr, d_len16, P<uint32_t>(ctx->x_units));
-            int rc = scan_u32(ctx, ctx->stream, ctx->scan_sums, P<uint32_t>(ctx->x_units), nr, P<uint32_t>(ctx->x_off4), nullptr);
+            Lookback lb;
+            int rc = lookback_state(ctx, ctx->stream, ctx->scan_sums, scan_tiles(nr), 1, &lb);
             if (rc) return rc;
-            d_off4 = P<uint32_t>(ctx->x_off4);
-        }
-        vtx_k_expand_reads<<<blocks_for(nr, 256), 256, 0, ctx->stream>>>(nr, d_len16, d_off4, P<uint64_t>(ctx->x_read_off), P<uint32_t>(ctx->x_read_len));
+            vtx_k_expand_dense<<<scan_tiles(nr), kScanThreads, 0, ctx->stream>>>(nr, d_len16, lb, P<uint64_t>(ctx->x_read_off),
+                                                                                P<uint32_t>(ctx->x_read_len));
+        } else {
+            vtx_k_expand_reads<<<blocks_for(nr, 256), 256, 0, ctx->stream>>>(nr, d_len16, d_off4, P<uint64_t>(ctx->x_read_off), P<uint32_t>(ctx->x_read_len));
+        }
         CK(cudaGetLastError());
     }
     d.read_off = P<uint64_t>(ctx->x_read_off); d.read_len = P<uint32_t>(ctx->x_read_len);
diff --git a/vartrix_b200/csrc/vtx_pipeline.cuh b/vartrix_b200/csrc/vtx_pipeline.cuh
--- a/vartrix_b200/csrc/vtx_pipeline.cuh
+++ b/vartrix_b200/csrc/vtx_pipeline.cuh
@@ -1,6 +1,7 @@
 #pragma once
 #include <cstdint>
 #include <cuda_runtime.h>
+#include <cuda/atomic>
 #include "vtx_sw.cuh"
 #include "vtx_sw_split.cuh"
 #include "vtx_sw_fold.cuh"
@@ -91,11 +92,8 @@
     read_col[r] = col;
 }
 
-__global__ void vtx_k_read_units(uint32_t n_reads, const uint16_t* __restrict__ read_len, uint32_t* __restrict__ units)
-{
-    const uint32_t r = blockIdx.x * blockDim.x + threadIdx.x;
-    if (r < n_reads) units[r] = ((uint32_t(read_len[r]) + 1) / 2 + 3) / 4;
-}
+__device__ __forceinline__ uint32_t read_units(uint32_t len) { return ((len + 1) / 2 + 3) / 4; }
+
 __global__ void vtx_k_expand_reads(uint32_t n_reads, const uint16_t* __restrict__ read_len, const uint32_t* __restrict__ off4,
                                    uint64_t* __restrict__ read_off, uint32_t* __restrict__ read_len32)
 {
@@ -105,31 +103,11 @@
     read_len32[r] = read_len[r];
 }
 
-__global__ void vtx_k_cand_filter(uint64_t n_cand, const uint32_t* __restrict__ cand_read,
-                                  const int32_t* __restrict__ read_col, const uint64_t* __restrict__ read_umi_key,
-                                  int use_umi, uint32_t* __restrict__ keep, unsigned long long* __restrict__ metrics)
-{
-    const uint64_t c = uint64_t(blockIdx.x) * blockDim.x + threadIdx.x;
-    bool miss_cb = false, miss_umi = false, ok = false;
-    if (c < n_cand) {
-        const uint32_t r = cand_read ? cand_read[c] : uint32_t(c);
-        if (read_col[r] < 0) miss_cb = true;
-        else if (use_umi && read_umi_key[r] == kNoUmi) miss_umi = true;
-        else ok = true;
-        keep[c] = ok ? 1u : 0u;
-    }
-    __shared__ uint32_t s_cnt[3];
-    if (threadIdx.x < 3) s_cnt[threadIdx.x] = 0;
-    __syncthreads();
-    const uint32_t b0 = __ballot_sync(0xffffffffu, miss_cb), b1 = __ballot_sync(0xffffffffu, miss_umi),
-                   b2 = __ballot_sync(0xffffffffu, ok);
-    if ((threadIdx.x & 31) == 0) {
-        if (b0) atomicAdd(&s_cnt[0], uint32_t(__popc(b0)));
-        if (b1) atomicAdd(&s_cnt[1], uint32_t(__popc(b1)));
-        if (b2) atomicAdd(&s_cnt[2], uint32_t(__popc(b2)));
-    }
-    __syncthreads();
-    if (threadIdx.x < 3 && s_cnt[threadIdx.x]) atomicAdd(metrics + threadIdx.x, (unsigned long long)s_cnt[threadIdx.x]);
+__device__ __forceinline__ int cand_rule(int32_t col, const uint64_t* __restrict__ read_umi_key, uint32_t r, int use_umi)
+{
+    if (col < 0) return 0;
+    if (use_umi && read_umi_key[r] == kNoUmi) return 1;
+    return 2;
 }
 
 __device__ __forceinline__ uint32_t locus_of_cand(const uint64_t* __restrict__ cand_start, uint32_t n_loci, uint64_t c)
@@ -140,20 +118,6 @@
         if (cand_start[mid] <= c) lo = mid; else hi = mid;
     }
     return lo;
-}
-
-__global__ void vtx_k_compact(uint64_t n_cand, const uint32_t* __restrict__ cand_read,
-                              const uint32_t* __restrict__ keep, const uint32_t* __restrict__ pidx,
-                              const int32_t* __restrict__ read_col, const uint64_t* __restrict__ read_umi_key,
-                              int use_umi, uint32_t* __restrict__ pair_read, uint32_t* __restrict__ pair_col,
-                              uint64_t* __restrict__ pair_umi)
-{
-    const uint64_t c = uint64_t(blockIdx.x) * blockDim.x + threadIdx.x;
-    if (c >= n_cand || !keep[c]) return;
-    const uint32_t p = pidx[c], r = cand_read ? cand_read[c] : uint32_t(c);
-    pair_read[p] = r;
-    pair_col[p] = uint32_t(read_col[r]);
-    if (use_umi) pair_umi[p] = read_umi_key[r];
 }
 
 __global__ void vtx_k_pair_start(uint32_t n_loci, const uint64_t* __restrict__ cand_start,
@@ -407,64 +371,68 @@
     atomicAdd(ccnt + size_t(cs) * 4 + k, 1u);
 }
 
-__global__ void vtx_k_finalize(uint32_t n_slots_ub, const uint32_t* __restrict__ n_pairs_ptr, int mode,
-                               const uint32_t* __restrict__ cslot_col, const uint32_t* __restrict__ ccnt,
-                               uint32_t* __restrict__ keep)
-{
-    const uint32_t q = blockIdx.x * blockDim.x + threadIdx.x;
-    if (q >= n_slots_ub) return;
-    uint32_t k = 0;
-    if (q < *n_pairs_ptr && cslot_col[q] != kInvalid) {
-        if (mode == 0) {
-            const uint4 c = reinterpret_cast<const uint4*>(ccnt)[q];
-            k = (c.x > 0 || c.y > 0) ? 1u : 0u;
-        } else k = 1u;
-    }
-    keep[q] = k;
-}
-
 struct ResultArrays {
     uint32_t* row; uint32_t* col; uint32_t* ref_cnt; uint32_t* alt_cnt; uint32_t* unk_cnt;
     double* val; double* val2;
 };
 
-__global__ void vtx_k_emit(uint32_t n_slots_ub, int mode, const uint32_t* __restrict__ keep,
-                           const uint32_t* __restrict__ oidx, const unsigned long long* __restrict__ res_base,
-                           const uint32_t* __restrict__ cslot_col, const uint32_t* __restrict__ cslot_locus,
-                           const uint32_t* __restrict__ locus_row, const uint32_t* __restrict__ ccnt, ResultArrays out)
-{
-    const uint32_t q = blockIdx.x * blockDim.x + threadIdx.x;
-    if (q >= n_slots_ub || !keep[q]) return;
-    const uint64_t o = *res_base + oidx[q];
-    const uint4 c = reinterpret_cast<const uint4*>(ccnt)[q];
-    const uint32_t r = c.x, a = c.y, u = c.z;
-    out.row[o] = locus_row[cslot_locus[q]];
-    out.col[o] = cslot_col[q];
-    out.ref_cnt[o] = r; out.alt_cnt[o] = a; out.unk_cnt[o] = u;
-    double v = 0.0, v2 = 0.0;
-    if (mode == 0) v = (r > 0 && a > 0) ? 3.0 : (a > 0 ? 2.0 : 1.0);
-    else if (mode == 2) v = double(a) / (double(r) + double(a) + double(u));
-    else { v = double(a); v2 = double(r); }
-    out.val[o] = v; out.val2[o] = v2;
-}
-
 __global__ void vtx_k_add_u64(unsigned long long* dst, const unsigned long long* __restrict__ src, int n)
 {
     if (blockIdx.x == 0 && int(threadIdx.x) < n) dst[threadIdx.x] += src[threadIdx.x];
 }
 
-__global__ void vtx_k_bump(unsigned long long* res_n, const uint32_t* __restrict__ total, unsigned long long* cum_host)
-{
-    if (threadIdx.x == 0 && blockIdx.x == 0) {
-        const unsigned long long n = *res_n + (total ? *total : 0u);
-        *res_n = n;
-        if (cum_host) *cum_host = n;
-    }
+__global__ void vtx_k_bump(const unsigned long long* __restrict__ res_n, unsigned long long* cum_host)
+{
+    if (threadIdx.x == 0 && blockIdx.x == 0) *cum_host = *res_n;
 }
 
 constexpr int kScanThreads = 256;
 constexpr int kScanItems = 8;
 constexpr int kScanTile = kScanThreads * kScanItems;
+
+constexpr unsigned long long kTileAgg = 1ull << 32, kTilePrefix = 2ull << 32;
+
+struct Lookback { unsigned long long* state; };
+
+__host__ __device__ inline size_t lookback_bytes(uint64_t tiles, uint32_t rows) { return size_t(8) * rows * (tiles + 1); }
+
+__device__ __forceinline__ uint32_t lookback_ticket(Lookback lb)
+{
+    __shared__ uint32_t s_tile;
+    if (threadIdx.x == 0) s_tile = atomicAdd(reinterpret_cast<unsigned int*>(lb.state + blockIdx.y), 1u);
+    __syncthreads();
+    return s_tile;
+}
+
+__device__ __forceinline__ unsigned long long* lookback_status(Lookback lb)
+{
+    return lb.state + gridDim.y + size_t(blockIdx.y) * gridDim.x;
+}
+
+__device__ uint32_t lookback_warp(unsigned long long* status, uint32_t tile, uint32_t agg)
+{
+    const int lane = threadIdx.x & 31;
+    if (tile == 0) {
+        if (lane == 0) cuda::atomic_ref<unsigned long long, cuda::thread_scope_device>(status[0]).store(kTilePrefix | agg, cuda::memory_order_release);
+        return 0;
+    }
+    if (lane == 0) cuda::atomic_ref<unsigned long long, cuda::thread_scope_device>(status[tile]).store(kTileAgg | agg, cuda::memory_order_release);
+    uint32_t excl = 0;
+    for (int64_t top = int64_t(tile) - 1;; top -= 32) {
+        const int64_t j = top - lane;
+        unsigned long long s;
+        do {
+            s = j >= 0 ? cuda::atomic_ref<unsigned long long, cuda::thread_scope_device>(status[j]).load(cuda::memory_order_acquire)
+                       : kTilePrefix;
+        } while (__any_sync(0xffffffffu, (s >> 32) == 0));
+        const uint32_t pre = __ballot_sync(0xffffffffu, (s >> 32) == 2);
+        const int stop = pre ? __ffs(pre) - 1 : 32;
+        excl += __reduce_add_sync(0xffffffffu, lane <= stop ? uint32_t(s) : 0u);
+        if (pre) break;
+    }
+    if (lane == 0) cuda::atomic_ref<unsigned long long, cuda::thread_scope_device>(status[tile]).store(kTilePrefix | (excl + agg), cuda::memory_order_release);
+    return excl;
+}
 
 __device__ __forceinline__ uint32_t block_exclusive_scan(uint32_t v, uint32_t* total)
 {
@@ -488,6 +456,69 @@
     *total = s_total;
     __syncthreads();
     return prefix;
+}
+
+__device__ __forceinline__ uint32_t lookback_scan(Lookback lb, uint32_t tile, uint32_t v, uint32_t* incl)
+{
+    __shared__ uint32_t s_excl;
+    uint32_t agg;
+    const uint32_t p = block_exclusive_scan(v, &agg);
+    if (threadIdx.x < 32) {
+        const uint32_t e = lookback_warp(lookback_status(lb), tile, agg);
+        if (threadIdx.x == 0) s_excl = e;
+    }
+    __syncthreads();
+    *incl = s_excl + agg;
+    return s_excl + p;
+}
+
+__global__ void __launch_bounds__(kScanThreads) vtx_k_scan(const uint32_t* __restrict__ in, uint64_t n, uint64_t stride,
+                                                           uint32_t* __restrict__ out, Lookback lb)
+{
+    const uint32_t tile = lookback_ticket(lb);
+    in += blockIdx.y * stride; out += blockIdx.y * stride;
+    const uint64_t base = uint64_t(tile) * kScanTile + uint64_t(threadIdx.x) * kScanItems;
+    uint32_t v[kScanItems], s = 0;
+#pragma unroll
+    for (int i = 0; i < kScanItems; ++i) { v[i] = (base + i < n) ? in[base + i] : 0; s += v[i]; }
+    uint32_t incl;
+    uint32_t p = lookback_scan(lb, tile, s, &incl);
+#pragma unroll
+    for (int i = 0; i < kScanItems; ++i) { if (base + i < n) out[base + i] = p; p += v[i]; }
+    if (tile == gridDim.x - 1 && threadIdx.x == 0) out[n] = incl;
+}
+
+__global__ void __launch_bounds__(kScanThreads) vtx_k_expand_dense(uint32_t n_reads, const uint16_t* __restrict__ read_len,
+                                                                   Lookback lb, uint64_t* __restrict__ read_off,
+                                                                   uint32_t* __restrict__ read_len32)
+{
+    __shared__ uint32_t s_v[kScanTile];
+    const uint32_t tile = lookback_ticket(lb);
+    const uint64_t t0 = uint64_t(tile) * kScanTile;
+    uint32_t len[kScanItems];
+#pragma unroll
+    for (int i = 0; i < kScanItems; ++i) {
+        const uint32_t j = i * kScanThreads + threadIdx.x;
+        len[i] = t0 + j < n_reads ? read_len[t0 + j] : 0u;
+        s_v[j] = read_units(len[i]);
+    }
+    __syncthreads();
+    uint4* mine = reinterpret_cast<uint4*>(s_v + threadIdx.x * kScanItems);
+    const uint4 a = mine[0], b = mine[1];
+    uint32_t incl;
+    uint32_t p = lookback_scan(lb, tile, a.x + a.y + a.z + a.w + b.x + b.y + b.z + b.w, &incl);
+    uint4 pa, pb;
+    pa.x = p; p += a.x; pa.y = p; p += a.y; pa.z = p; p += a.z; pa.w = p; p += a.w;
+    pb.x = p; p += b.x; pb.y = p; p += b.y; pb.z = p; p += b.z; pb.w = p;
+    mine[0] = pa; mine[1] = pb;
+    __syncthreads();
+#pragma unroll
+    for (int i = 0; i < kScanItems; ++i) {
+        const uint32_t j = i * kScanThreads + threadIdx.x;
+        if (t0 + j >= n_reads) break;
+        read_off[t0 + j] = uint64_t(s_v[j]) * 4;
+        read_len32[t0 + j] = len[i];
+    }
 }
 
 __global__ void __launch_bounds__(kScanThreads) vtx_k_scan_tiles(const uint32_t* __restrict__ in, uint64_t n,
@@ -519,26 +550,6 @@
     if (threadIdx.x == 0) *total_out = carry;
 }
 
-__global__ void __launch_bounds__(kScanThreads) vtx_k_scan_rows(const uint32_t* __restrict__ in, uint32_t* __restrict__ out,
-                                                                uint32_t n, uint32_t stride)
-{
-    const uint32_t* src = in + size_t(blockIdx.x) * stride;
-    uint32_t* dst = out + size_t(blockIdx.x) * stride;
-    uint32_t carry = 0;
-    for (uint32_t base = 0; base < n; base += kScanTile) {
-        const uint32_t i0 = base + threadIdx.x * kScanItems;
-        uint32_t v[kScanItems], sum = 0;
-#pragma unroll
-        for (int k = 0; k < kScanItems; ++k) { v[k] = (i0 + k < n) ? src[i0 + k] : 0; sum += v[k]; }
-        uint32_t total;
-        uint32_t p = carry + block_exclusive_scan(sum, &total);
-#pragma unroll
-        for (int k = 0; k < kScanItems; ++k) { if (i0 + k < n) dst[i0 + k] = p; p += v[k]; }
-        carry += total;
-    }
-    if (threadIdx.x == 0) dst[n] = carry;
-}
-
 __global__ void __launch_bounds__(kScanThreads) vtx_k_scan_add(uint32_t* __restrict__ out, uint64_t n,
                                                                const uint32_t* __restrict__ sums)
 {
@@ -548,4 +559,126 @@
     for (int i = 0; i < kScanItems; ++i) if (base + i < n) out[base + i] += add;
 }
 
-}
+struct TileFlags {
+    uint8_t flag[kScanTile];
+    uint32_t pos[kScanTile];
+};
+
+__device__ __forceinline__ uint32_t lookback_flags(Lookback lb, uint32_t tile, TileFlags& s)
+{
+    __syncthreads();
+    const uint2 f = reinterpret_cast<const uint2*>(s.flag)[threadIdx.x];
+    const uint32_t cnt = __popc(f.x) + __popc(f.y);
+    uint32_t incl;
+    uint32_t p = lookback_scan(lb, tile, cnt, &incl);
+    uint32_t q[kScanItems];
+#pragma unroll
+    for (int k = 0; k < kScanItems; ++k) { q[k] = p; p += ((k < 4 ? f.x : f.y) >> (8 * (k & 3))) & 1u; }
+    uint4* dst = reinterpret_cast<uint4*>(s.pos + threadIdx.x * kScanItems);
+    dst[0] = make_uint4(q[0], q[1], q[2], q[3]);
+    dst[1] = make_uint4(q[4], q[5], q[6], q[7]);
+    __syncthreads();
+    return incl;
+}
+
+__global__ void __launch_bounds__(kScanThreads) vtx_k_cand_compact(
+    uint64_t n_cand, const uint32_t* __restrict__ cand_read, const int32_t* __restrict__ read_col,
+    const uint64_t* __restrict__ read_umi_key, int use_umi, Lookback lb, uint32_t* __restrict__ pidx,
+    uint32_t* __restrict__ pair_read, uint32_t* __restrict__ pair_col, uint64_t* __restrict__ pair_umi,
+    unsigned long long* __restrict__ metrics)
+{
+    __shared__ TileFlags s;
+    __shared__ uint32_t s_cnt[3];
+    if (threadIdx.x < 3) s_cnt[threadIdx.x] = 0;
+    const uint32_t tile = lookback_ticket(lb);
+    const uint64_t t0 = uint64_t(tile) * kScanTile;
+    uint32_t rd[kScanItems]; int32_t col[kScanItems];
+    uint32_t cnt[3] = { 0, 0, 0 };
+#pragma unroll
+    for (int i = 0; i < kScanItems; ++i) {
+        const uint32_t j = i * kScanThreads + threadIdx.x;
+        const uint64_t c = t0 + j;
+        uint8_t keep = 0;
+        if (c < n_cand) {
+            rd[i] = cand_read ? cand_read[c] : uint32_t(c);
+            col[i] = read_col[rd[i]];
+            const int k = cand_rule(col[i], read_umi_key, rd[i], use_umi);
+            cnt[0] += k == 0; cnt[1] += k == 1; cnt[2] += k == 2;
+            keep = k == 2;
+        }
+        s.flag[j] = keep;
+    }
+#pragma unroll
+    for (int k = 0; k < 3; ++k) {
+        const uint32_t w = __reduce_add_sync(0xffffffffu, cnt[k]);
+        if ((threadIdx.x & 31) == 0 && w) atomicAdd(&s_cnt[k], w);
+    }
+    const uint32_t incl = lookback_flags(lb, tile, s);
+#pragma unroll
+    for (int i = 0; i < kScanItems; ++i) {
+        const uint32_t j = i * kScanThreads + threadIdx.x;
+        const uint64_t c = t0 + j;
+        if (c >= n_cand) break;
+        const uint32_t p = s.pos[j];
+        pidx[c] = p;
+        if (s.flag[j]) {
+            pair_read[p] = rd[i];
+            pair_col[p] = uint32_t(col[i]);
+            if (use_umi) pair_umi[p] = read_umi_key[rd[i]];
+        }
+    }
+    if (tile == gridDim.x - 1 && threadIdx.x == 0) pidx[n_cand] = incl;
+    if (threadIdx.x < 3 && s_cnt[threadIdx.x]) atomicAdd(metrics + threadIdx.x, (unsigned long long)s_cnt[threadIdx.x]);
+}
+
+__global__ void __launch_bounds__(kScanThreads) vtx_k_finalize_emit(
+    uint32_t n_slots_ub, const uint32_t* __restrict__ n_pairs_ptr, int mode, const uint32_t* __restrict__ cslot_col,
+    const uint32_t* __restrict__ cslot_locus, const uint32_t* __restrict__ locus_row, const uint32_t* __restrict__ ccnt,
+    Lookback lb, unsigned long long* res_n, unsigned long long* cum_host, ResultArrays out)
+{
+    __shared__ TileFlags s;
+    __shared__ unsigned long long s_base;
+    if (threadIdx.x == 0) s_base = *res_n;
+    const uint32_t tile = lookback_ticket(lb);
+    const uint32_t n_slots = min(n_slots_ub, *n_pairs_ptr);
+    const uint64_t t0 = uint64_t(tile) * kScanTile;
+    uint32_t col[kScanItems];
+    uint4 cnt[kScanItems];
+#pragma unroll
+    for (int i = 0; i < kScanItems; ++i) {
+        const uint32_t j = i * kScanThreads + threadIdx.x;
+        const uint64_t q = t0 + j;
+        uint8_t keep = 0;
+        col[i] = q < n_slots ? cslot_col[q] : kInvalid;
+        if (col[i] != kInvalid) {
+            cnt[i] = reinterpret_cast<const uint4*>(ccnt)[q];
+            keep = mode != 0 || cnt[i].x > 0 || cnt[i].y > 0;
+        }
+        s.flag[j] = keep;
+    }
+    const uint32_t incl = lookback_flags(lb, tile, s);
+    const unsigned long long base = s_base;
+#pragma unroll
+    for (int i = 0; i < kScanItems; ++i) {
+        const uint32_t j = i * kScanThreads + threadIdx.x;
+        const uint64_t q = t0 + j;
+        if (!s.flag[j]) continue;
+        const uint64_t o = base + s.pos[j];
+        const uint32_t r = cnt[i].x, a = cnt[i].y, u = cnt[i].z;
+        out.row[o] = locus_row[cslot_locus[q]];
+        out.col[o] = col[i];
+        out.ref_cnt[o] = r; out.alt_cnt[o] = a; out.unk_cnt[o] = u;
+        double v = 0.0, v2 = 0.0;
+        if (mode == 0) v = (r > 0 && a > 0) ? 3.0 : (a > 0 ? 2.0 : 1.0);
+        else if (mode == 2) v = double(a) / (double(r) + double(a) + double(u));
+        else { v = double(a); v2 = double(r); }
+        out.val[o] = v; out.val2[o] = v2;
+    }
+    if (tile == gridDim.x - 1 && threadIdx.x == 0) {
+        const unsigned long long n = base + incl;
+        *res_n = n;
+        if (cum_host) *cum_host = n;
+    }
+}
+
+}
```

New measurement: 180.2 million (median of 6 runs). +1.8%, better.
